# wen-yuan-zhang/Fast-Learning-NeRF

Hardware: AMD Instinct MI355X
Metric: training rays/sec (Lego-like 800x800, 64+128 samples) + PSNR@N-iters (higher is better)
Workload: dtype f32; 1 GPU; nerf-ours Lego full 800x800 (BASELINE configs[1]), SURVEY 8(d) throughput protocol: 4096 uniformly drawn rays per GPU per step, 64+128 samples, use_viewdirs, white_bkgd, perturb=1, U[0,1) targets, random-init nets, leaf-error table on, fp32-width bf16x6 kernels, plain backward (FASTNERF_COMPACT=0); parallelism=dp1, math_mode=bf16x6, backward=plain (every sample)

## Files before the change

fast-learning-nerf_amd/_lib.py:

```python
import ctypes as C
import os

import torch

HERE = os.path.dirname(os.path.abspath(__file__))
LIB_PATH = os.environ.get('FASTNERF_LIB') or os.path.join(HERE, 'libfastnerf.so')

P = C.c_void_p
I = C.c_int
L = C.c_int64
F = C.c_float
D = C.c_double
U64 = C.c_uint64



class StepArgs(C.Structure):
    _fields_ = (
        [('n', L)] + [(k, P) for k in ('rays_o', 'rays_d', 'target', 't_rand', 'u', 'noise0', 'noise1')]
        + [('seed0', U64), ('seed1', U64), ('leaf_tag', P), ('table', P), ('net_floats', L)]
        + [(k, P) for k in ('params', 'grads', 'adam_m', 'adam_v', 'packed_fwd_c', 'packed_bwd_c', 'packed_fwd_f', 'packed_bwd_f',
                            'rays11', 'z0', 'raw0', 'act0', 'rgb0', 'disp0', 'acc0', 'w0', 'depth0',
                            'z1', 'z_samples', 'z_std', 'raw1', 'act1', 'rgb1', 'disp1', 'acc1', 'w1', 'depth1',
                            'g_rgb', 'g_rgb0', 'loss2', 'draw_ws', 'act_ws', 'dact_ws', 'partial_ws', 'live_ws', 'counts')]
        + [(k, D) for k in ('focal', 'lr', 'beta1', 'beta2', 'eps')]
        + [(k, F) for k in ('near_plane', 'far_plane', 'grad_scale')]
        + [(k, I) for k in ('math_mode', 'N_samples', 'N_importance', 'lindisp', 'perturb', 'white_bkgd', 'ndc', 'H', 'W', 'live',
                            'fwd_flags', 'max_leaves', 'adam_t')]
        + [('occ', P), ('occ_counts', P)])


class OccGrid(C.Structure):
    _fields_ = [('words', P), ('lo', F * 3), ('inv', F * 3), ('n', C.c_int32 * 3), ('outside_occupied', C.c_int32)]


OCC_MAX_LEVELS = 8


class OccCascade(C.Structure):
    _fields_ = [('levels', C.c_int32), ('reserved', C.c_int32), ('level', OccGrid * OCC_MAX_LEVELS)]


STEP_FORWARD, STEP_BWD_FINE, STEP_BWD_COARSE, STEP_UPDATE = 1, 2, 4, 8

SIGNATURES = {
    'fastnerf_version': (I, []),
    'fastnerf_last_error': (C.c_char_p, []),
    'fastnerf_device_cus': (I, []),
    'fastnerf_gen_rays': (I, [I, I, F, F, F, F, P, P, P, P]),
    'fastnerf_gen_rays_pixels': (I, [L, P, P, F, F, F, F, P, P, P]),
    'fastnerf_ndc_rays': (I, [L, I, I, D, F, P, P, P, P, P]),
    'fastnerf_pack_rays': (I, [L, P, P, F, F, I, I, I, D, P, P]),
    'fastnerf_sample_coarse': (I, [L, I, P, I, I, P, U64, P, P]),
    'fastnerf_posenc': (I, [L, I, P, P, P]),
    'fastnerf_mlp_pack': (I, [P, P, P, P]),
    'fastnerf_mlp_fwd': (I, [L, I, P, P, P, P, P, P, P]),
    'fastnerf_mlp_bwd_partial_floats': (L, []),
    'fastnerf_mlp_bwd': (I, [L, I, P, P, P, P, P, P, P, P]),
    'fastnerf_raw2outputs_fwd': (I, [L, I, P, P, P, P, I, P, P, P, P, P, P]),
    'fastnerf_raw2outputs_bwd': (I, [L, I, P, P, P, P, I, P, P, P]),
    'fastnerf_raw2outputs_bwd_full': (I, [L, I, P, P, P, P, I, P, P, P, P, P, P, P, P, P]),
    'fastnerf_sample_pdf_merge': (I, [L, I, I, P, P, I, P, U64, P, P, P, P]),
    'fastnerf_sample_pdf': (I, [L, I, I, P, P, I, P, U64, P, P]),
    'fastnerf_mse_leafmax': (I, [L, P, P, P, F, P, P, P, P, I, P, P]),
    'fastnerf_adam_step': (I, [L, P, P, P, P, D, D, D, D, I, P]),
    'fastnerf_net_floats': (L, [I, I]),
    'fastnerf_mlp_act_floats': (L, [I, L]),
    'fastnerf_mlp_pack_ex': (I, [I, P, P, P, P]),
    'fastnerf_mlp_fwd_ex': (I, [I, L, I, P, P, P, P, P, P, P]),
    'fastnerf_mlp_bwd_ex': (I, [I, L, I, P, P, P, P, P, P, P, P]),
    'fastnerf_mlp_bf16_floats': (L, [I, I, L]),
    'fastnerf_mlp_bf16_partial_floats': (L, []),
    'fastnerf_mlp_bf16_pack': (I, [I, P, P, P, P]),
    'fastnerf_mlp_bf16_fwd': (I, [I, L, I, P, P, P, P, P, P, P]),
    'fastnerf_mlp_bf16_bwd': (I, [I, L, I, P, P, P, P, P, P, P, P]),
    'fastnerf_render_rays_fwd': (I, [I, L, I, I, P, I, I, I, I, P, P, P, P, U64, U64, P, P, P, P] + [P] * 18 + [P]),
    'fastnerf_render_rays_fwd_ex': (I, [I, L, I, I, P, I, I, I, I, P, P, P, P, U64, U64, P, P, P, P] + [P] * 18 + [I, P]),
    'fastnerf_mlp_bf16_fwd_flags': (I, [I, L, I, P, P, P, P, P, I, P]),
    'fastnerf_mlp_fwd_flags_ex': (I, [I, L, I, P, P, P, P, P, I, P]),
    'fastnerf_render_rays_bwd': (I, [I, L, I, I, P, I] + [P] * 20),
    'fastnerf_pp_intersect_sphere': (I, [L, P, P, P, P]),
    'fastnerf_pp_fg_depths': (I, [L, I, F, P, I, P, U64, P, P]),
    'fastnerf_pp_sample_pdf_merge': (I, [L, I, I, P, P, I, P, U64, P, P, P]),
    'fastnerf_pp_perturb_samples': (I, [L, I, P, P, U64, P, P]),
    'fastnerf_pp_sample_pdf': (I, [L, I, I, P, P, I, P, U64, P, P]),
    'fastnerf_pp_depth2pts_outside': (I, [L, I, P, P, P, P, P, P]),
    'fastnerf_pp_composite_fwd': (I, [L, I, I, P, P, P, P, P, P, P, P, P]),
    'fastnerf_pp_composite_bwd': (I, [L, I, I, P, P, P, P, P, P, P, P]),
    'fastnerf_pp_gen_rays': (I, [I, I, P, P, P, P, P]),
    'fastnerf_leaf_sumcount': (I, [L, P, P, P, I, P, P, P]),
    'fastnerf_tree_adjust_mean': (L, [P, P, P, I, D]),
    'fastnerf_tree_create': (P, [I, I, I, I]),
    'fastnerf_tree_destroy': (None, [P]),
    'fastnerf_tree_num_leaves': (I, [P, I]),
    'fastnerf_tree_max_leaves': (I, [P]),
    'fastnerf_tree_min_area': (D, [P, I]),
    'fastnerf_tree_get_leaves': (I, [P, I, P]),
    'fastnerf_tree_set_leaves': (I, [P, I, I, P, D]),
    'fastnerf_tree_leaf_plan': (I, [P, I, D, I, P]),
    'fastnerf_tree_adjust': (L, [P, P, I, D]),
    'fastnerf_tree_epoch_plan': (L, [P, D, I, P, P]),
    'fastnerf_epoch_rays': (I, [L, I, P, P, P, P, I, I, I, F, F, F, F, U64, I] + [P] * 10 + [P]),
    'fastnerf_epoch_rays_shard': (I, [L, I, P, P, P, P, I, I, I, F, F, F, F, U64, I] + [P] * 5 + [L, I, I] + [P] * 5 + [P]),
    'fastnerf_epoch_shard_rows': (L, [L, L, I, I]),
    'fastnerf_gauss_noise': (I, [L, F, U64, P, P]),
    'fastnerf_compact_ws_ints': (L, [L]),
    'fastnerf_compact_live': (I, [L, P, P, P, P, P]),
    'fastnerf_mlp_bf16_fwd_live': (I, [I, L, I, P, P, P, P, P, P, P, P]),
    'fastnerf_mlp_bf16_bwd_live': (I, [I, L, I, P, P, P, P, P, P, P, P, P, P]),
    'fastnerf_mlp_fwd_live_ex': (I, [I, L, I, P, P, P, P, P, P, P, P]),
    'fastnerf_mlp_bwd_live_ex': (I, [I, L, I, P, P, P, P, P, P, P, P, P, P]),
    'fastnerf_render_rays_bwd_live': (I, [I, L, I, I, P, I] + [P] * 22 + [P]),
    'fastnerf_mlp_x6_packed_floats': (L, [I, I]),
    'fastnerf_mlp_x6_pack': (I, [I, P, P, P, P]),
    'fastnerf_mlp_x6_fwd': (I, [I, L, I, P, P, P, P, P, P, I, P]),
    'fastnerf_mlp_x6_bwd': (I, [I, L, I, P, P, P, P, P, P, P, P]),
    'fastnerf_mlp_x6_fwd_live': (I, [I, L, I, P, P, P, P, P, P, P, P]),
    'fastnerf_mlp_x6_bwd_live': (I, [I, L, I, P, P, P, P, P, P, P, P, P, P]),
    'fastnerf_step_args_size': (L, []),
    'fastnerf_train_step': (I, [C.POINTER(StepArgs), I, P]),
    'fastnerf_comm_unique_id': (I, [C.c_char_p]),
    'fastnerf_comm_init': (I, [C.POINTER(P), C.c_char_p, I, I]),
    'fastnerf_comm_destroy': (I, [P]),
    'fastnerf_allreduce_grads': (I, [P, P, L, C.c_float, P]),
    'fastnerf_allreduce_leaf_table': (I, [P, P, L, P]),
    'fastnerf_allreduce_leaf_sumcount': (I, [P, P, P, L, P]),
    'fastnerf_leaf_table_reset': (I, [P, L, P]),
    'fastnerf_leaf_table_read': (I, [P, P, L, P]),
    'fastnerf_grid_points': (I, [L, L, P, L, P, L, P, L, P, P]),
    'fastnerf_grid_sigma': (I, [L, P, P, P]),
    'fastnerf_mc_ws_bytes': (L, [L, L, L]),
    'fastnerf_mc_count': (I, [P, L, L, L, F, P, P, P]),
    'fastnerf_mc_emit': (I, [P, L, L, L, F, P, P, P, P]),
    'fastnerf_mc_tables': (I, [P, P]),
    'fastnerf_occ_words': (L, [L, L, L]),
    'fastnerf_occ_build': (I, [P, L, L, L, F, I, P, P, P]),
    'fastnerf_occ_from_mask': (I, [P, L, L, L, P, P]),
    'fastnerf_occ_query': (I, [C.POINTER(OccGrid), L, P, P, P]),
    'fastnerf_occ_classify': (I, [C.POINTER(OccGrid), L, I, P, P, P, P, P, P, P]),
    'fastnerf_occ_query_cascade': (I, [C.POINTER(OccCascade), L, P, P, P]),
    'fastnerf_occ_classify_cascade': (I, [C.POINTER(OccCascade), L, I, P, P, P, P, P, P, P]),
    'fastnerf_occ_cell_points': (I, [C.POINTER(OccGrid), L, L, U64, P, P]),
    'fastnerf_occ_update': (I, [P, P, L, L, L, L, L, F, F, I, P, P, P, P]),
    'fastnerf_mlp_fwd_list_ex': (I, [I, L, I, P, P, P, P, P, P, P, I, P]),
    'fastnerf_mlp_bf16_fwd_list': (I, [I, L, I, P, P, P, P, P, P, P, I, P]),
    'fastnerf_mlp_x6_fwd_list': (I, [I, L, I, P, P, P, P, P, P, P, I, P]),
    'fastnerf_render_rays_fwd_occ': (I, [I, L, I, I, P, I, I, I, I, P, P, U64, U64, P, P, P, P, C.POINTER(OccGrid), P, P] + [P] * 16 + [I, P]),
    'fastnerf_render_rays_fwd_occ_cascade': (I, [I, L, I, I, P, I, I, I, I, P, P, U64, U64, P, P, P, P, C.POINTER(OccCascade), P, P] + [P] * 16 + [I, P]),
    'fastnerf_mlp_sigma_grad_ws_floats': (L, [I, L]),
    'fastnerf_mlp_sigma_grad': (I, [I, I, L, I, P, P, P, P, P, P, P, P, P]),
}

_lib = None


def lib():
    global _lib
    if _lib is None:
        if not os.path.exists(LIB_PATH):
            raise RuntimeError(
                f'{LIB_PATH} not found: build it with `python -c "import __graft_entry__ as g; g.build()"` '
                '(the HIP path has no CPU fallback)')
        l = C.CDLL(LIB_PATH)
        for name, (res, args) in SIGNATURES.items():
            fn = getattr(l, name)
            fn.restype = res
            fn.argtypes = args
        if l.fastnerf_step_args_size() != C.sizeof(StepArgs):
            raise RuntimeError('fn_step_args: the ctypes mirror does not match the library (stale libfastnerf.so?)')
        _lib = l
    return _lib


def check(rc, what):
    if rc is None or rc < 0:
        msg = lib().fastnerf_last_error()
        raise RuntimeError(f'{what} failed ({rc}): {msg.decode() if msg else "?"}')
    return rc


def ptr(t):
    if t is None:
        return None
    assert t.is_contiguous(), 'tensor must be contiguous'
    return t.data_ptr()


def stream():
    return torch.cuda.current_stream().cuda_stream


def require_gpu(*tensors):
    for t in tensors:
        if t is not None and not t.is_cuda:
            raise RuntimeError('fastnerf ops run on the GPU only (no CPU fallback): got a CPU tensor')
```

fast-learning-nerf_amd/csrc/mlp_bwd_dw.hip:

```cpp
#include "mlp_common.h"

int fn_launch_dx(int mm, int grid, hipStream_t st, int64_t P, const float* draw, const float* act, const float* params, const float* packed_bwd,
                 float* dact, const NetLayout& L, const int* live_idx, const int* live_cnt);

#define DW_MT 32

template <int WO, int WI, int TO, int TI, bool BIAS, bool RANK1>
__global__ void __launch_bounds__(WO * WI * 64, WO * WI / 4)
mlp_bwd_dw_kernel(int64_t P, const float* __restrict__ dY, int ldy, const float* __restrict__ X, int ldx,
                  const float* __restrict__ draw , float* __restrict__ partial_w,
                  float* __restrict__ partial_b, float* __restrict__ partial_r, const int* __restrict__ live_idx,
                  const int* __restrict__ live_cnt) {
  if (live_idx) P = (int64_t)__builtin_amdgcn_readfirstlane(*live_cnt);
  constexpr int NO = WO * TO * 32, KI = WI * TI * 32;
  constexpr int NTD = WO * WI * 64;
  constexpr int STAGE = DW_MT * (NO + KI) + DW_MT;
  extern __shared__ __attribute__((aligned(16))) float smem[];
  const int tid = threadIdx.x;
  const int lane = tid & 63;
  const int wave = __builtin_amdgcn_readfirstlane(tid >> 6);
  const int wo = wave / WI, wi = wave % WI;
  const int64_t ntile_all = (P + DW_MT - 1) / DW_MT;
  const int64_t per = (ntile_all + gridDim.x - 1) / gridDim.x;
  const int64_t t0 = blockIdx.x * per;
  int64_t t1 = t0 + per;
  if (t1 > ntile_all) t1 = ntile_all;

  f32x16 acc[TO][TI];
#pragma unroll
  for (int a = 0; a < TO; ++a)
#pragma unroll
    for (int b = 0; b < TI; ++b)
#pragma unroll
      for (int r = 0; r < 16; ++r) acc[a][b][r] = 0.f;
  float bsum = 0.f, rsum = 0.f;

  constexpr int YV = (DW_MT * NO / 4 + NTD - 1) / NTD;
  constexpr int XV = (DW_MT * KI / 4 + NTD - 1) / NTD;
  static_assert(DW_MT * NO % 4 == 0 && DW_MT * KI % 4 == 0 && NO <= NTD && KI <= NTD, "stage split");
  float4 ry[YV], rx[XV];
  float rda = 0.f;

  auto load_stage = [&](int64_t t) {
    const int64_t pbase = t * DW_MT;
#pragma unroll
    for (int i = 0; i < YV; ++i) {
      const int e = (i * NTD + tid) * 4;
      const int m = e / NO, c = e % NO;
      const int64_t p = pbase + m;
      ry[i] = (e < DW_MT * NO && p < P) ? *reinterpret_cast<const float4*>(dY + p * ldy + c)
                                        : make_float4(0.f, 0.f, 0.f, 0.f);
    }
#pragma unroll
    for (int i = 0; i < XV; ++i) {
      const int e = (i * NTD + tid) * 4;
      const int m = e / KI, c = e % KI;
      const int64_t p = pbase + m;
      rx[i] = (e < DW_MT * KI && p < P) ? *reinterpret_cast<const float4*>(X + p * ldx + c)
                                        : make_float4(0.f, 0.f, 0.f, 0.f);
    }
    if (RANK1 && tid < DW_MT) {
      const int64_t p = pbase + tid;
      rda = (p < P) ? draw[(live_idx ? (int64_t)live_idx[p] : p) * 4 + 3] : 0.f;
    }
  };
  auto store_stage = [&](float* st) {
#pragma unroll
    for (int i = 0; i < YV; ++i)
      if ((i * NTD + tid) * 4 < DW_MT * NO) *reinterpret_cast<float4*>(st + (i * NTD + tid) * 4) = ry[i];
#pragma unroll
    for (int i = 0; i < XV; ++i)
      if ((i * NTD + tid) * 4 < DW_MT * KI) *reinterpret_cast<float4*>(st + DW_MT * NO + (i * NTD + tid) * 4) = rx[i];
    if (RANK1 && tid < DW_MT) st[DW_MT * (NO + KI) + tid] = rda;
  };

  if (t0 < t1) {
    load_stage(t0);
    store_stage(smem);
  }
  __syncthreads();
  for (int64_t t = t0; t < t1; ++t) {
    float* cur = smem + ((t - t0) & 1) * STAGE;
    float* nxt = smem + (((t - t0) & 1) ^ 1) * STAGE;
    if (t + 1 < t1) load_stage(t + 1);
    const float* Ys = cur;
    const float* Xs = cur + DW_MT * NO;
    {
      float fa0[TO], fb0[TI], fa1[TO], fb1[TI];
      auto ldf = [&](float (&a)[TO], float (&b)[TI], int k2) {
        const int m = k2 * 2 + (lane >> 5);
#pragma unroll
        for (int i = 0; i < TO; ++i) a[i] = Ys[m * NO + (wo * TO + i) * 32 + (lane & 31)];
#pragma unroll
        for (int j = 0; j < TI; ++j) b[j] = Xs[m * KI + (wi * TI + j) * 32 + (lane & 31)];
      };
      auto mm = [&](const float (&a)[TO], const float (&b)[TI]) {
#pragma unroll
        for (int i = 0; i < TO; ++i)
#pragma unroll
          for (int j = 0; j < TI; ++j) acc[i][j] = mfma(a[i], b[j], acc[i][j]);
      };
      ldf(fa0, fb0, 0);
#pragma unroll
      for (int k2 = 0; k2 < DW_MT / 2; k2 += 2) {
        ldf(fa1, fb1, k2 + 1);
        __builtin_amdgcn_sched_barrier(0);
        mm(fa0, fb0);
        __builtin_amdgcn_sched_barrier(0);
        if (k2 + 2 < DW_MT / 2) ldf(fa0, fb0, k2 + 2);
        __builtin_amdgcn_sched_barrier(0);
        mm(fa1, fb1);
        __builtin_amdgcn_sched_barrier(0);
      }
    }
    if (BIAS) {
      if (tid < NO) {
#pragma unroll 8
        for (int m = 0; m < DW_MT; ++m) bsum += Ys[m * NO + tid];
      }
    }
    if (RANK1) {
      if (tid < KI) {
        const float* da = cur + DW_MT * (NO + KI);
#pragma unroll 8
        for (int m = 0; m < DW_MT; ++m) rsum = fmaf(da[m], Xs[m * KI + tid], rsum);
      }
    }
    if (t + 1 < t1) store_stage(nxt);
    __syncthreads();
  }
  float* pw = partial_w + (int64_t)blockIdx.x * NO * KI;
#pragma unroll
  for (int i = 0; i < TO; ++i)
#pragma unroll
    for (int j = 0; j < TI; ++j)
#pragma unroll
      for (int r = 0; r < 16; ++r) {
        const int o = (wo * TO + i) * 32 + crow(r, lane);
        const int c = (wi * TI + j) * 32 + (lane & 31);
        pw[(int64_t)o * KI + c] = acc[i][j][r];
      }
  if (BIAS && tid < NO) partial_b[(int64_t)blockIdx.x * NO + tid] = bsum;
  if (RANK1 && tid < KI) partial_r[(int64_t)blockIdx.x * KI + tid] = rsum;
}

template <int WO, int WI, int TO, int TI, bool BIAS, bool RANK1, int CTI2 = 0, int CTO2 = 0>
__device__ __forceinline__ void dw6_body(const int64_t P, const float* __restrict__ dY, const float* __restrict__ X,
                                         const float* __restrict__ draw, float* __restrict__ partial_w, float* __restrict__ partial_b,
                                         float* __restrict__ partial_r, const int* __restrict__ live_idx,
                                         const float* __restrict__ X2, const float* __restrict__ dY2, const int wg, const int nwg) {
  constexpr int NO = WO * TO * 32, KI = WI * TI * 32;
  constexpr int CTO = WO * TO, CTI = WI * TI, NTILE = CTO + CTI;
  constexpr int NW = WO * WI;
  constexpr int TPW = (NTILE + NW - 1) / NW;
  extern __shared__ __attribute__((aligned(16))) uint4 S6[];
  float* const DA = reinterpret_cast<float*>(S6 + 2 * NTILE * 192);
  const int tid = threadIdx.x;
  const int lane = tid & 63;
  const int wave = __builtin_amdgcn_readfirstlane(tid >> 6);
  const int wo = wave / WI, wi = wave % WI;
  const int64_t nq_all = (P + 15) / 16;
  const int64_t per = (nq_all + nwg - 1) / nwg;
  const int64_t q0 = wg * per;
  int64_t q1 = q0 + per;
  if (q1 > nq_all) q1 = nq_all;
  const int nq = (int)(q1 - q0);
  int64_t Pend = q1 * 16;
  if (Pend > P) Pend = P;

  f32x16 acc[TO][TI];
#pragma unroll
  for (int a = 0; a < TO; ++a)
#pragma unroll
    for (int b = 0; b < TI; ++b)
#pragma unroll
      for (int r = 0; r < 16; ++r) acc[a][b][r] = 0.f;
  float ssum[TPW];
#pragma unroll
  for (int k = 0; k < TPW; ++k) ssum[k] = 0.f;

  constexpr int CTI1 = CTI - CTI2, KI1 = CTI1 * 32, KI2 = CTI2 * 32;
  static_assert(!(RANK1 && CTI2), "the rank-1 row is taken over X only");
  constexpr int CTO1 = CTO - CTO2, NO1 = CTO1 * 32, NO2 = CTO2 * 32;
  static_assert(!(RANK1 && CTO2) && !(CTI2 && CTO2), "one second tensor per job");
  const float* tsrc[TPW];
  bool tisy[TPW], tis2[TPW];
  constexpr bool KNOWN = (CTO % NW == 0) && (NTILE % NW == 0) && CTO2 == 0 && CTI2 == 0;
#pragma unroll
  for (int k = 0; k < TPW; ++k) {
    const int t = k * NW + wave;
    tisy[k] = KNOWN ? (k * NW < CTO) : (t < CTO);
    tis2[k] = (CTI2 > 0 && t >= CTO + CTI1) || (CTO2 > 0 && t >= CTO1 && t < CTO);
    tsrc[k] = tisy[k] ? (tis2[k] ? dY2 + q0 * (16 * NO2) + (t - CTO1) * 32 : dY + q0 * (16 * NO1) + t * 32)
                      : (tis2[k] ? X2 + q0 * (16 * KI2) + (t - CTO - CTI1) * 32 : X + q0 * (16 * KI1) + (t - CTO) * 32);
  }
  const int relmax = (int)(Pend - q0 * 16) - 1;
  const int col = lane & 31, half8 = (lane >> 5) * 8;
  const unsigned boffy = (unsigned)(half8 * NO1 + col) * 4u, boffy2 = (unsigned)(half8 * NO2 + col) * 4u,
                 boffx = (unsigned)(half8 * KI1 + col) * 4u, boffx2 = (unsigned)(half8 * KI2 + col) * 4u;
  struct Raw { float v[TPW][8]; };
  auto ldb = [](const float* base, unsigned byte_off) __attribute__((always_inline)) -> float {
    return *reinterpret_cast<const float*>(reinterpret_cast<const char*>(base) + byte_off);
  };
  auto load_raw = [&](Raw& r, int st, auto whole) __attribute__((always_inline)) {
    if constexpr (decltype(whole)::value) {
#pragma unroll
      for (int k = 0; k < TPW; ++k) {
        const int t = k * NW + wave;
        if (NTILE % NW == 0 || t < NTILE) {
          if (tisy[k] && CTO2 > 0 && tis2[k]) {
            const float* b = tsrc[k] + (int64_t)st * (16 * NO2);
#pragma unroll
            for (int e = 0; e < 8; ++e) r.v[k][e] = ldb(b, boffy2 + (unsigned)(e * NO2 * 4));
          } else if (tisy[k]) {
            const float* b = tsrc[k] + (int64_t)st * (16 * NO1);
#pragma unroll
            for (int e = 0; e < 8; ++e) r.v[k][e] = ldb(b, boffy + (unsigned)(e * NO1 * 4));
          } else if (CTI2 > 0 && tis2[k]) {
            const float* b = tsrc[k] + (int64_t)st * (16 * KI2);
#pragma unroll
            for (int e = 0; e < 8; ++e) r.v[k][e] = ldb(b, boffx2 + (unsigned)(e * KI2 * 4));
          } else {
            const float* b = tsrc[k] + (int64_t)st * (16 * KI1);
#pragma unroll
            for (int e = 0; e < 8; ++e) r.v[k][e] = ldb(b, boffx + (unsigned)(e * KI1 * 4));
          }
        }
      }
    } else {
      unsigned row[8];
#pragma unroll
      for (int e = 0; e < 8; ++e) { const int rr = st * 16 + half8 + e; row[e] = (unsigned)(rr < relmax ? rr : relmax); }
#pragma unroll
      for (int k = 0; k < TPW; ++k) {
        const int t = k * NW + wave;
        if (NTILE % NW == 0 || t < NTILE) {
#pragma unroll
          for (int e = 0; e < 8; ++e)
            r.v[k][e] = ldb(tsrc[k], (row[e] * (unsigned)(tisy[k] ? (tis2[k] ? NO2 : NO1) : (tis2[k] ? KI2 : KI1)) + (unsigned)col) * 4u);
        }
      }
    }
  };
  const int* const li = live_idx ? live_idx : reinterpret_cast<const int*>(draw);
  auto load_ix = [&](int st) __attribute__((always_inline)) -> int64_t {
    const int rr = st * 16 + (lane & 15);
    const int64_t p = q0 * 16 + (rr < relmax ? rr : relmax);
    const int64_t lv = li[p];
    return live_idx ? lv : p;
  };
  auto split_store = [&](const Raw& r, int buf, int st, auto whole) __attribute__((always_inline)) {
    const int nv = relmax + 1 - (st * 16 + half8);
#pragma unroll
    for (int k = 0; k < TPW; ++k) {
      const int t = k * NW + wave;
      if (NTILE % NW == 0 || t < NTILE) {
        float v[8];
#pragma unroll
        for (int e = 0; e < 8; ++e) v[e] = r.v[k][e];
        if constexpr (!decltype(whole)::value) {
#pragma unroll
          for (int e = 0; e < 8; ++e) v[e] = e < nv ? v[e] : 0.f;
        }
        uint4 h, m, l;
        uint4* d = S6 + ((buf * NTILE + t) * 3) * 64 + lane;
        split3_frag(make_float4(v[0], v[1], v[2], v[3]), make_float4(v[4], v[5], v[6], v[7]), h, m, l);
        d[0] = h; d[64] = m; d[128] = l;
        if (BIAS && (KNOWN ? (k * NW < CTO) : (t < CTO1))) ssum[k] += ((v[0] + v[1]) + (v[2] + v[3])) + ((v[4] + v[5]) + (v[6] + v[7]));
        if (RANK1 && (KNOWN ? (k * NW >= CTO) : (t >= CTO))) {
          const float4 d0 = *reinterpret_cast<const float4*>(DA + (st & 1) * 16 + half8);
          const float4 d1 = *reinterpret_cast<const float4*>(DA + (st & 1) * 16 + half8 + 4);
          const float da[8] = {d0.x, d0.y, d0.z, d0.w, d1.x, d1.y, d1.z, d1.w};
#pragma unroll
          for (int e = 0; e < 8; ++e) ssum[k] = fmaf(da[e], v[e], ssum[k]);
        }
      }
    }
  };
  auto multiply = [&](int buf) __attribute__((always_inline)) {
    const uint4* Sb = S6 + buf * NTILE * 192 + lane;
    uint4 a[TO][3];
#pragma unroll
    for (int i = 0; i < TO; ++i)
#pragma unroll
      for (int pl = 0; pl < 3; ++pl) a[i][pl] = Sb[((wo * TO + i) * 3 + pl) * 64];
    constexpr int PA[6] = {2, 0, 1, 1, 0, 0}, PB[6] = {0, 2, 1, 0, 1, 0};
    constexpr int JP = TI >= 2 ? 2 : 1;
#pragma unroll
    for (int j0 = 0; j0 < TI; j0 += JP) {
      uint4 b[JP][3];
#pragma unroll
      for (int jj = 0; jj < JP; ++jj)
#pragma unroll
        for (int pl = 0; pl < 3; ++pl)
          if (j0 + jj < TI) b[jj][pl] = Sb[((CTO + wi * TI + j0 + jj) * 3 + pl) * 64];
#pragma unroll
      for (int t = 0; t < 6; ++t)
#pragma unroll
        for (int jj = 0; jj < JP; ++jj)
#pragma unroll
          for (int i = 0; i < TO; ++i)
            if (j0 + jj < TI) acc[i][j0 + jj] = mfma_bf16(a[i][PA[t]], b[jj][PB[t]], acc[i][j0 + jj]);
    }
  };
  auto publish = [&]() __attribute__((always_inline)) {
    asm volatile("s_waitcnt lgkmcnt(0)\n\ts_barrier" ::: "memory");
  };

  if (nq > 0) {
    constexpr std::true_type WHOLE{};
    constexpr std::false_type ANY{};
    Raw r0, r1;
    load_raw(r0, 0, ANY);
    load_raw(r1, 1, ANY);
    float dr0 = 0.f, dr1 = 0.f;
    int64_t ix0 = 0, ix1 = 0;
    const bool da_lane = RANK1 && wave == 0 && lane < 16;
    if (da_lane) {
      DA[lane] = draw[load_ix(0) * 4 + 3];
      DA[16 + lane] = draw[load_ix(1) * 4 + 3];
      dr0 = draw[load_ix(2) * 4 + 3];
      dr1 = draw[load_ix(3) * 4 + 3];
      ix0 = load_ix(4);
      ix1 = load_ix(5);
    }
    if (RANK1) publish();
    split_store(r0, 0, 0, ANY);
    load_raw(r0, 2, ANY);
    publish();
    auto mix = [&](auto sync) __attribute__((always_inline)) {
      if constexpr (KNOWN && !RANK1) interleave6<0, TO * TI * 6, TPW * 4 * 11 + (BIAS ? 8 : 0), decltype(sync)::value>();
    };
    auto pair = [&](int d, auto whole) __attribute__((always_inline)) {
      const int st = 2 * d;
      if (da_lane) { DA[lane] = dr0; dr0 = draw[ix0 * 4 + 3]; ix0 = load_ix(st + 6); }
      multiply(0);
      split_store(r1, 1, st + 1, whole);
      mix(std::integral_constant<int, 1>{});
      load_raw(r1, st + 3, whole);
      publish();
      if (da_lane) { DA[16 + lane] = dr1; dr1 = draw[ix1 * 4 + 3]; ix1 = load_ix(st + 7); }
      multiply(1);
      split_store(r0, 0, st + 2, whole);
      mix(std::integral_constant<int, 2>{});
      load_raw(r0, st + 4, whole);
      publish();
    };
    const int n2 = (nq + 1) / 2;
    const int nwhole = (relmax + 1) / 16;
    int dmain = nwhole >= 5 ? (nwhole - 3) / 2 : 0;
    if (dmain > n2) dmain = n2;
#pragma unroll 1
    for (int d = 0; d < dmain; ++d) pair(d, WHOLE);
#pragma unroll 1
    for (int d = dmain; d < n2; ++d) pair(d, ANY);
  }
  float* pw = partial_w + (int64_t)wg * NO * KI;
#pragma unroll
  for (int i = 0; i < TO; ++i)
#pragma unroll
    for (int j = 0; j < TI; ++j)
#pragma unroll
      for (int r = 0; r < 16; ++r) {
        const int o = (wo * TO + i) * 32 + crow(r, lane);
        const int c = (wi * TI + j) * 32 + (lane & 31);
        pw[(int64_t)o * KI + c] = acc[i][j][r];
      }
  if (BIAS || RANK1) {
#pragma unroll
    for (int k = 0; k < TPW; ++k) {
      const int t = k * NW + wave;
      if (NTILE % NW == 0 || t < NTILE) {
        const float sv = ssum[k] + __shfl_xor(ssum[k], 32, 64);
        if (lane < 32) {
          if (BIAS && t < CTO1) partial_b[(int64_t)wg * NO1 + t * 32 + lane] = sv;
          if (RANK1 && t >= CTO) partial_r[(int64_t)wg * KI + (t - CTO) * 32 + lane] = sv;
        }
      }
    }
  }
}

template <int WO, int WI, int TO, int TI, bool BIAS, bool RANK1, int CTI2 = 0, int CTO2 = 0>
__global__ void __launch_bounds__(WO * WI * 64, WO * WI / 4)
mlp_bwd_dw6_kernel(int64_t P, const float* __restrict__ dY, const float* __restrict__ X,
                   const float* __restrict__ draw, float* __restrict__ partial_w, float* __restrict__ partial_b,
                   float* __restrict__ partial_r, const int* __restrict__ live_idx, const int* __restrict__ live_cnt,
                   const float* __restrict__ X2 = nullptr, const float* __restrict__ dY2 = nullptr) {
  if (live_idx) P = (int64_t)__builtin_amdgcn_readfirstlane(*live_cnt);
  dw6_body<WO, WI, TO, TI, BIAS, RANK1, CTI2, CTO2>(P, dY, X, draw, partial_w, partial_b, partial_r, live_idx, X2, dY2, (int)blockIdx.x,
                                                    (int)gridDim.x);
}

#define DW_QMAX 256
__host__ __device__ static inline int dw_trunk_chunks(int64_t P, int ncu) {
  const int unit = ncu >= 8 ? ncu / 8 : 1;
  const int64_t nq = (P + 15) / 16;
  int64_t k = (nq + (int64_t)unit * DW_QMAX - 1) / ((int64_t)unit * DW_QMAX);
  k = k < 1 ? 1 : (k > 8 ? 8 : k);
  return unit * (int)k;
}
struct DwTrunk {
  const float* dY[8];
  const float* X[8];
  float* pw[8];
  float* pb[8];
};
__global__ void __launch_bounds__(512, 2)
mlp_bwd_dw6_trunk_kernel(int64_t P, DwTrunk J, const float* __restrict__ draw, float* __restrict__ partial_r,
                         const int* __restrict__ live_idx, const int* __restrict__ live_cnt, int ncu) {
  if (live_idx) P = (int64_t)__builtin_amdgcn_readfirstlane(*live_cnt);
  const int nact = dw_trunk_chunks(P, ncu);
  if ((int)blockIdx.x >= nact) return;
  const int job = (int)blockIdx.y;
  if (job == 7)
    dw6_body<4, 2, 2, 4, true, true>(P, J.dY[7], J.X[7], draw, J.pw[7], J.pb[7], partial_r, live_idx, nullptr, nullptr, (int)blockIdx.x, nact);
  else
    dw6_body<4, 2, 2, 4, true, false>(P, J.dY[job], J.X[job], nullptr, J.pw[job], J.pb[job], nullptr, live_idx, nullptr, nullptr,
                                      (int)blockIdx.x, nact);
}

__global__ void __launch_bounds__(128) head_grads_kernel(int64_t P, const float* __restrict__ draw,
                                                          const float* __restrict__ hv,
                                                          float* __restrict__ partial, const int* __restrict__ live_idx,
                                                          const int* __restrict__ live_cnt) {
  const int k = threadIdx.x;
  if (live_idx) P = *live_cnt;
  auto dptr = [&](int64_t q) { return draw + (live_idx ? (int64_t)live_idx[q] : q) * 4; };
  const int64_t per = (P + gridDim.x - 1) / gridDim.x;
  const int64_t pa = blockIdx.x * per;
  int64_t pb = pa + per;
  if (pb > P) pb = P;
  float s0 = 0.f, s1 = 0.f, s2 = 0.f, sb = 0.f;
  int64_t p = pa;
  constexpr int NF = 16;
  for (; p + NF <= pb; p += NF) {
    float4 d[NF];
    float h[NF];
#pragma unroll
    for (int i = 0; i < NF; ++i) {
      d[i] = *reinterpret_cast<const float4*>(dptr(p + i));
      h[i] = hv[(p + i) * 128 + k];
    }
#pragma unroll
    for (int i = 0; i < NF; ++i) {
      s0 = fmaf(d[i].x, h[i], s0); s1 = fmaf(d[i].y, h[i], s1); s2 = fmaf(d[i].z, h[i], s2);
      if (k < 4) sb += (k == 0) ? d[i].x : (k == 1) ? d[i].y : (k == 2) ? d[i].z : d[i].w;
    }
  }
  for (; p < pb; ++p) {
    const float4 d = *reinterpret_cast<const float4*>(dptr(p));
    const float h = hv[p * 128 + k];
    s0 = fmaf(d.x, h, s0); s1 = fmaf(d.y, h, s1); s2 = fmaf(d.z, h, s2);
    if (k < 4) sb += (k == 0) ? d.x : (k == 1) ? d.y : (k == 2) ? d.z : d.w;
  }
  float* o = partial + (int64_t)blockIdx.x * 388;
  o[k] = s0; o[128 + k] = s1; o[256 + k] = s2;
  if (k < 4) o[384 + k] = sb;
}

struct RedSeg {
  int64_t src;
  int64_t wg_stride;
  int64_t dst;
  int nwg, rows, cols, ld, valid_cols;
  int dyn;
};
#define MAX_SEGS 32
struct RedTable {
  RedSeg s[MAX_SEGS];
  int n;
};

__global__ void __launch_bounds__(256) reduce_all_kernel(RedTable tab, const float* __restrict__ partial,
                                                          float* __restrict__ grads, int64_t P, const int* __restrict__ live_cnt, int ncu) {
  RedSeg sg = tab.s[blockIdx.y];
  if (sg.dyn) {
    if (live_cnt) P = (int64_t)*live_cnt;
    const int n = dw_trunk_chunks(P, ncu);
    sg.nwg = n < sg.nwg ? n : sg.nwg;
  }
  const int64_t total = (int64_t)sg.rows * sg.cols;
  const float* src = partial + sg.src;
  for (int64_t e = blockIdx.x * (int64_t)blockDim.x + threadIdx.x; e < total; e += (int64_t)gridDim.x * blockDim.x) {
    const int r = (int)(e / sg.cols), c = (int)(e % sg.cols);
    if (c >= sg.valid_cols) continue;
    constexpr int RS = 16;
    float a[RS];
#pragma unroll
    for (int i = 0; i < RS; ++i) a[i] = 0.f;
    int w = 0;
    for (; w + RS <= sg.nwg; w += RS) {
#pragma unroll
      for (int i = 0; i < RS; ++i) a[i] += src[(int64_t)(w + i) * sg.wg_stride + e];
    }
#pragma unroll
    for (int i = 0; i < RS - 1; ++i)
      if (w + i < sg.nwg) a[i] += src[(int64_t)(w + i) * sg.wg_stride + e];
#pragma unroll
    for (int h = RS / 2; h >= 1; h >>= 1)
#pragma unroll
      for (int i = 0; i < h; ++i) a[i] += a[i + h];
    grads[sg.dst + (int64_t)r * sg.ld + c] = a[0];
  }
}

struct DwJobDesc { int NO, KI, bias, rank1; };
static DwJobDesc dw_job(int j, int pe_pad) {
  switch (j) {
    case 0: return {256, pe_pad, 1, 0};
    case 8: return {256, pe_pad, 0, 0};
    case 9: return {256, 256, 1, 1};
    case 10: return {128, 256, 1, 0};
    case 11: return {128, 32, 0, 0};
    default: return {256, 256, 1, 0};
  }
}
#define HEAD_MAX_WG 1024
static int64_t dw_job_floats(int j, int pe_pad) {
  const DwJobDesc d = dw_job(j, pe_pad);
  return (int64_t)d.NO * d.KI + (d.bias ? d.NO : 0) + (d.rank1 ? d.KI : 0);
}
static int64_t dw_job_base(int j, int ncu, int pe_pad) {
  static const int order[12] = {0, 8, 1, 2, 3, 4, 5, 6, 7, 9, 10, 11};
  int64_t o = 0;
  for (int i = 0; i < 12; ++i) {
    if (order[i] == j) return o;
    o += dw_job_floats(order[i], pe_pad) * ncu;
  }
  return o;
}
extern "C" int64_t fastnerf_mlp_bwd_partial_floats(void) {
  return dw_job_base(12, num_cus(), 96) + (int64_t)HEAD_MAX_WG * 388;
}

template <int WO, int WI, int TO, int TI, bool BIAS, bool RANK1, int MM = MM_F32, int CTI2 = 0, int CTO2 = 0>
static int launch_dw(int64_t P, const float* dY, int ldy, const float* X, int ldx, const float* draw, float* base,
                     int nwg, hipStream_t st, const int* live_idx = nullptr, const int* live_cnt = nullptr,
                     const float* X2 = nullptr, const float* dY2 = nullptr) {
  constexpr int NO = WO * TO * 32, KI = WI * TI * 32;
  float* pw = base;
  float* pb = base + (int64_t)nwg * NO * KI;
  float* pr = pb + (BIAS ? (int64_t)nwg * (NO - CTO2 * 32) : 0);
  if constexpr (MM == MM_X6) {
    if (ldy != NO - CTO2 * 32 || ldx != KI - CTI2 * 32 || (CTI2 > 0) != (X2 != nullptr) || (CTO2 > 0) != (dY2 != nullptr)) {
      fn::set_error("launch_dw: the bf16x6 dW kernel needs ld == width (and X2 / dY2 exactly when CTI2 / CTO2 > 0)");
      return -1;
    }
    constexpr int lds6 = 2 * (WO * TO + WI * TI) * 3 * 1024 + 128;
    auto kern6 = mlp_bwd_dw6_kernel<WO, WI, TO, TI, BIAS, RANK1, CTI2, CTO2>;
    static bool attr6 = false;
    if (!attr6) {
      FN_HIP(hipFuncSetAttribute(reinterpret_cast<const void*>(kern6), hipFuncAttributeMaxDynamicSharedMemorySize, lds6));
      attr6 = true;
    }
    hipLaunchKernelGGL(kern6, dim3(nwg), dim3(WO * WI * 64), lds6, st, P, dY, X, draw, pw, pb, pr, live_idx, live_cnt, X2, dY2);
    FN_LAUNCH_CHECK();
    return 0;
  } else {
    static_assert(MM == MM_F32 && CTI2 == 0 && CTO2 == 0, "two-tensor jobs exist for the bf16x6 dW kernel only");
    constexpr int STAGE = DW_MT * (NO + KI) + DW_MT;
    const size_t lds = 2 * STAGE * sizeof(float);
    auto kern = mlp_bwd_dw_kernel<WO, WI, TO, TI, BIAS, RANK1>;
    static bool attr = false;
    if (!attr) {
      FN_HIP(hipFuncSetAttribute(reinterpret_cast<const void*>(kern), hipFuncAttributeMaxDynamicSharedMemorySize, (int)lds));
      attr = true;
    }
    hipLaunchKernelGGL(kern, dim3(nwg), dim3(WO * WI * 64), lds, st, P, dY, ldy, X, ldx, draw, pw, pb, pr, live_idx, live_cnt);
    FN_LAUNCH_CHECK();
    return 0;
  }
}

static void add_seg(RedTable& T, int64_t src, int64_t wg_stride, int nwg, int rows, int cols, int64_t dst, int ld,
                    int valid_cols, int dyn = 0) {
  RedSeg& s = T.s[T.n++];
  s.src = src; s.wg_stride = wg_stride; s.nwg = nwg; s.rows = rows; s.cols = cols; s.dst = dst; s.ld = ld;
  s.valid_cols = valid_cols; s.dyn = dyn;
}

template <int MM>
static int bwd_launch_t(int kind, int64_t n, int S, const float* draw, const float* act, const float* params,
                      const float* packed_bwd, float* dact, float* partial, float* grads, const int* live_idx,
                      const int* live_cnt, fn_stream_t stream) {
  constexpr int MW = MM;
  const NetLayout& L = layout_of(kind);
  const int PEP = L.pe_pad;
  hipStream_t st = fn::S(stream);
  const int64_t P = n * S;
  const int64_t ntiles = (P + TM - 1) / TM;
  const int ncu = num_cus();
  int grid = ncu * WG_PER_CU;
  if (ntiles < grid) grid = (int)ntiles;
  if (int rc_dx = fn_launch_dx(MM, grid, st, P, draw, act, params, packed_bwd, dact, L, live_idx, live_cnt)) return rc_dx;

  const int nwg = ncu;
  RedTable T;
  T.n = 0;
  int rc;
  const float* a_pe = act + act_pe(P, PEP);
  auto region = [&](int j) { return partial + dw_job_base(j, ncu, PEP); };
  auto segs = [&](int j, int64_t dstW, int ld, int validc, int64_t dstB, int64_t dstR, int dyn = 0) {
    const DwJobDesc d = dw_job(j, PEP);
    const int64_t b = dw_job_base(j, ncu, PEP);
    add_seg(T, b, (int64_t)d.NO * d.KI, nwg, d.NO, d.KI, dstW, ld, validc, dyn);
    int64_t o = b + (int64_t)nwg * d.NO * d.KI;
    if (d.bias) { add_seg(T, o, d.NO, nwg, 1, d.NO, dstB, d.NO, d.NO, dyn); o += (int64_t)nwg * d.NO; }
    if (d.rank1) add_seg(T, o, d.KI, nwg, 1, d.KI, dstR, d.KI, d.KI, dyn);
  };
  if constexpr (MW == MM_X6) {
    if (PEP == 64) rc = launch_dw<8, 2, 2, 1, true, false, MW, 0, 8>(P, dact + dact_y(P, 0), 256, a_pe, 64, nullptr, region(0), nwg, st, live_idx, live_cnt, nullptr, dact + dact_y(P, 5));
    else rc = launch_dw<8, 1, 2, 3, true, false, MW, 0, 8>(P, dact + dact_y(P, 0), 256, a_pe, 96, nullptr, region(0), nwg, st, live_idx, live_cnt, nullptr, dact + dact_y(P, 5));
    if (rc) return rc;
    const int64_t b0 = dw_job_base(0, ncu, PEP);
    add_seg(T, b0, (int64_t)512 * PEP, nwg, 256, PEP, L.LW[0], L.in_pe, L.in_pe);
    add_seg(T, b0 + (int64_t)256 * PEP, (int64_t)512 * PEP, nwg, 256, PEP, L.LW[5], 256 + L.in_pe, L.in_pe);
    add_seg(T, b0 + (int64_t)nwg * 512 * PEP, 256, nwg, 1, 256, L.LB[0], 256, 256);
  } else {
    if (PEP == 64) rc = launch_dw<4, 1, 2, 2, true, false, MW>(P, dact + dact_y(P, 0), 256, a_pe, 64, nullptr, region(0), nwg, st, live_idx, live_cnt);
    else rc = launch_dw<4, 1, 2, 3, true, false, MW>(P, dact + dact_y(P, 0), 256, a_pe, 96, nullptr, region(0), nwg, st, live_idx, live_cnt);
    if (rc) return rc;
    segs(0, L.LW[0], L.in_pe, L.in_pe, L.LB[0], 0);
  }
  if constexpr (MW != MM_X6) {
    for (int l = 1; l < 8; ++l) {
      if ((rc = launch_dw<4, 2, 2, 4, true, false, MW>(P, dact + dact_y(P, l), 256, act + act_h(P, PEP, l - 1), 256, nullptr, region(l), nwg, st, live_idx, live_cnt))) return rc;
      segs(l, L.LW[l] + (l == 5 ? L.in_pe : 0), l == 5 ? 256 + L.in_pe : 256, 256, L.LB[l], 0);
    }
  }
  if constexpr (MW != MM_X6) {
    if (PEP == 64) rc = launch_dw<4, 1, 2, 2, false, false, MW>(P, dact + dact_y(P, 5), 256, a_pe, 64, nullptr, region(8), nwg, st, live_idx, live_cnt);
    else rc = launch_dw<4, 1, 2, 3, false, false, MW>(P, dact + dact_y(P, 5), 256, a_pe, 96, nullptr, region(8), nwg, st, live_idx, live_cnt);
    if (rc) return rc;
    segs(8, L.LW[5], 256 + L.in_pe, L.in_pe, 0, 0);
  }
  if constexpr (MW == MM_X6) {
    DwTrunk J;
    for (int l = 1; l <= 8; ++l) {
      const int j = l < 8 ? l : 9;
      J.dY[l - 1] = l < 8 ? dact + dact_y(P, l) : dact + dact_feat(P);
      J.X[l - 1] = act + act_h(P, PEP, l - 1);
      J.pw[l - 1] = region(j);
      J.pb[l - 1] = region(j) + (int64_t)nwg * 256 * 256;
    }
    float* pr = J.pb[7] + (int64_t)nwg * 256;
    constexpr int lds6 = 2 * 16 * 3 * 1024 + 128;
    static bool attr_t = false;
    if (!attr_t) {
      FN_HIP(hipFuncSetAttribute(reinterpret_cast<const void*>(mlp_bwd_dw6_trunk_kernel), hipFuncAttributeMaxDynamicSharedMemorySize, lds6));
      attr_t = true;
    }
    hipLaunchKernelGGL(mlp_bwd_dw6_trunk_kernel, dim3(dw_trunk_chunks(P, ncu), 8), dim3(512), lds6, st, P, J, draw, pr, live_idx, live_cnt, ncu);
    FN_LAUNCH_CHECK();
    for (int l = 1; l < 8; ++l) segs(l, L.LW[l] + (l == 5 ? L.in_pe : 0), l == 5 ? 256 + L.in_pe : 256, 256, L.LB[l], 0, 1);
    segs(9, L.FW, 256, 256, L.FB, L.AW, 1);
  } else {
    if ((rc = launch_dw<4, 2, 2, 4, true, true, MW>(P, dact + dact_feat(P), 256, act + act_h(P, PEP, 7), 256, draw, region(9), nwg, st, live_idx, live_cnt))) return rc;
    segs(9, L.FW, 256, 256, L.FB, L.AW);
  }
  if constexpr (MW == MM_X6) {
    if ((rc = launch_dw<4, 3, 1, 3, true, false, MW, 1, 0>(P, dact + dact_yv(P), 128, act + act_feat(P, PEP), 256, nullptr, region(10), nwg, st,
                                                     live_idx, live_cnt, act + act_vpe(P, PEP), nullptr))) return rc;
    const int64_t b10 = dw_job_base(10, ncu, PEP);
    add_seg(T, b10, 128 * 288, nwg, 128, 288, L.VW, 283, 283);
    add_seg(T, b10 + (int64_t)nwg * 128 * 288, 128, nwg, 1, 128, L.VB, 128, 128);
  } else {
    if ((rc = launch_dw<2, 4, 2, 2, true, false, MW>(P, dact + dact_yv(P), 128, act + act_feat(P, PEP), 256, nullptr, region(10), nwg, st, live_idx, live_cnt))) return rc;
    segs(10, L.VW, 283, 256, L.VB, 0);
    if ((rc = launch_dw<4, 1, 1, 1, false, false, MW>(P, dact + dact_yv(P), 128, act + act_vpe(P, PEP), 32, nullptr, region(11), nwg, st, live_idx, live_cnt))) return rc;
    segs(11, L.VW + 256, 283, 27, 0, 0);
  }
  {
    const int hg = HEAD_MAX_WG;
    const int64_t hb = dw_job_base(12, ncu, PEP);
    hipLaunchKernelGGL(head_grads_kernel, dim3(hg), dim3(128), 0, st, P, draw, act + act_hv(P, PEP), partial + hb, live_idx, live_cnt);
    FN_LAUNCH_CHECK();
    add_seg(T, hb, 388, hg, 1, 388, L.RW, 388, 387);
    add_seg(T, hb + 387, 388, hg, 1, 1, L.AB, 1, 1);
  }
  hipLaunchKernelGGL(reduce_all_kernel, dim3(256, T.n), dim3(256), 0, st, T, partial, grads, P, live_cnt, ncu);
  FN_LAUNCH_CHECK();
  return 0;
}
static int bwd_launch(int kind, int64_t n, int S, const float* draw, const float* act, const float* params,
                      const float* packed_bwd, float* dact, float* partial, float* grads, const int* live_idx,
                      const int* live_cnt, fn_stream_t stream, int mm = MM_F32) {
  return mm == MM_X6 ? bwd_launch_t<MM_X6>(kind, n, S, draw, act, params, packed_bwd, dact, partial, grads, live_idx, live_cnt, stream)
                     : bwd_launch_t<MM_F32>(kind, n, S, draw, act, params, packed_bwd, dact, partial, grads, live_idx, live_cnt, stream);
}
extern "C" int fastnerf_mlp_bwd_ex(int kind, int64_t n, int S, const float* draw, const float* act,
                                   const float* params, const float* packed_bwd, float* dact, float* partial,
                                   float* grads, fn_stream_t stream) {
  FN_CHECK_ARG(kind >= 0 && kind <= 2 && n > 0 && S >= 1, "kind in 0..2, n>0, S>=1");
  FN_CHECK_ARG(draw && act && params && packed_bwd && dact && partial && grads, "null pointer");
  return bwd_launch(kind, n, S, draw, act, params, packed_bwd, dact, partial, grads, nullptr, nullptr, stream);
}
extern "C" int fastnerf_mlp_bwd_live_ex(int kind, int64_t n, int S, const float* draw, const float* act,
                                        const float* params, const float* packed_bwd, float* dact, float* partial,
                                        float* grads, const int32_t* live_idx, const int32_t* live_cnt,
                                        fn_stream_t stream) {
  FN_CHECK_ARG(kind >= 0 && kind <= 2 && n > 0 && S >= 1, "kind in 0..2, n>0, S>=1");
  FN_CHECK_ARG(draw && act && params && packed_bwd && dact && partial && grads && live_idx && live_cnt, "null pointer");
  return bwd_launch(kind, n, S, draw, act, params, packed_bwd, dact, partial, grads, live_idx, live_cnt, stream);
}
extern "C" int fastnerf_mlp_bwd(int64_t n, int S, const float* draw, const float* act, const float* params,
                                const float* packed_bwd, float* dact, float* partial, float* grads,
                                fn_stream_t stream) {
  return fastnerf_mlp_bwd_ex(0, n, S, draw, act, params, packed_bwd, dact, partial, grads, stream);
}

extern "C" int fastnerf_mlp_x6_bwd(int kind, int64_t n, int S, const float* draw, const float* act, const float* params,
                                   const float* packed_bwd, float* dact, float* partial, float* grads, fn_stream_t stream) {
  FN_CHECK_ARG(kind >= 0 && kind <= 2 && n > 0 && S >= 1, "kind in 0..2, n>0, S>=1");
  FN_CHECK_ARG(draw && act && params && packed_bwd && dact && partial && grads, "null pointer");
  return bwd_launch(kind, n, S, draw, act, params, packed_bwd, dact, partial, grads, nullptr, nullptr, stream, MM_X6);
}
extern "C" int fastnerf_mlp_x6_bwd_live(int kind, int64_t n, int S, const float* draw, const float* act, const float* params,
                                        const float* packed_bwd, float* dact, float* partial, float* grads,
                                        const int32_t* live_idx, const int32_t* live_cnt, fn_stream_t stream) {
  FN_CHECK_ARG(kind >= 0 && kind <= 2 && n > 0 && S >= 1, "kind in 0..2, n>0, S>=1");
  FN_CHECK_ARG(draw && act && params && packed_bwd && dact && partial && grads && live_idx && live_cnt, "null pointer");
  return bwd_launch(kind, n, S, draw, act, params, packed_bwd, dact, partial, grads, live_idx, live_cnt, stream, MM_X6);
}
```

fast-learning-nerf_amd/csrc/mlp_bwd_dx.hip:

```cpp
#include "mlp_common.h"

struct DxPre {
  unsigned mlo, mhi;
  float wan[4];
};
template <bool MASK, bool RANK1, bool L16 = false>
__device__ __forceinline__ DxPre dx_preload(const unsigned long long* __restrict__ maskw, const float* __restrict__ wa,
                                            int wn, int lane) {
  DxPre p;
  p.mlo = p.mhi = 0u;
  p.wan[0] = p.wan[1] = p.wan[2] = p.wan[3] = 0.f;
  if (MASK) {
    const unsigned long long w = maskw[lane];
    p.mlo = (unsigned)w;
    p.mhi = (unsigned)(w >> 32);
  }
  if (RANK1) {
    if constexpr (L16) {
#pragma unroll
      for (int ct = 0; ct < 4; ++ct) p.wan[ct] = wa[(wn * 4 + ct) * 16 + (lane & 15)];
    } else {
      p.wan[0] = wa[(wn * 2 + 0) * 32 + (lane & 31)];
      p.wan[1] = wa[(wn * 2 + 1) * 32 + (lane & 31)];
    }
  }
  return p;
}
template <bool MASK, bool RANK1>
__device__ __forceinline__ void epilogue_dx(const f32x4m (&acc)[4][4], float* Hs, const float* Es_dalpha, const DxPre& pre,
                                            float* __restrict__ dsave, int wm, int wn, int lane, int valid) {
  asm volatile("" : "+v"(lane));
  const unsigned mlo = pre.mlo, mhi = pre.mhi;
  float* colp[4][4];
  h_cols16<4>(Hs, wm, wn, lane, colp);
  const int hq = lane >> 4;
#pragma unroll
  for (int mt = 0; mt < 4; ++mt) {
#pragma unroll
    for (int ct = 0; ct < 4; ++ct) {
      const float wan = pre.wan[ct];
#pragma unroll
      for (int r = 0; r < 4; ++r) {
        float v = acc[mt][ct][r];
        if (RANK1) v = fmaf(Es_dalpha[wm * 64 + mt * 16 + 4 * hq + r], wan, v);
        if (MASK) {
          const int idx = (mt * 4 + ct) * 4 + r;
          const int keep = __builtin_amdgcn_sbfe(idx < 32 ? (int)mlo : (int)mhi, 31 - (idx & 31), 1);
          v = __int_as_float(__float_as_int(v) & keep);
        }
        H16_AT(colp, ct, mt, r) = v;
      }
    }
    __builtin_amdgcn_sched_barrier(0);
  }
}

template <bool MASK, bool RANK1>
__device__ __forceinline__ void epilogue_dx(const f32x16 (&acc)[2][2], float* Hs, const float* Es_dalpha,
                                            const DxPre& pre, float* __restrict__ dsave, int wm, int wn, int lane,
                                            int valid) {
  asm volatile("" : "+v"(lane));
  const unsigned mlo = pre.mlo, mhi = pre.mhi;
  float* colp[2][8];
  h_cols<2>(Hs, wm, wn, lane, colp);
#pragma unroll
  for (int nt = 0; nt < 2; ++nt) {
    const int n = (wn * 2 + nt) * 32 + (lane & 31);
    const float wan = pre.wan[nt];
#pragma unroll
    for (int mt = 0; mt < 2; ++mt) {
#pragma unroll
      for (int r = 0; r < 16; ++r) {
        const int m = wm * 64 + mt * 32 + crow(r, lane);
        float v = acc[mt][nt][r];
        if (RANK1) v = fmaf(Es_dalpha[m], wan, v);
        if (MASK) {
          const int idx = (nt * 2 + mt) * 16 + r;
          const int keep = __builtin_amdgcn_sbfe(idx < 32 ? (int)mlo : (int)mhi, 31 - (idx & 31), 1);
          v = __int_as_float(__float_as_int(v) & keep);
        }
        H_AT(colp, nt, mt, r) = v;
        if (dsave != nullptr && m < valid) dsave[(unsigned)(m * 256 + n)] = v;
      }
      __builtin_amdgcn_sched_barrier(0);
    }
  }
}

template <int MM = MM_F32>
__global__ void __launch_bounds__(NTHR, 2 * NTHR / 512 * WG_PER_CU)
mlp_bwd_dx_kernel(int64_t P, const float* __restrict__ draw, const float* __restrict__ act,
                  const float* __restrict__ params, const float* __restrict__ packed_t, float* __restrict__ dact,
                  NetLayout lay, unsigned* __restrict__ sched, const int* __restrict__ live_idx,
                  const int* __restrict__ live_cnt) {
  const int64_t PL = P;
  if (live_idx) P = (int64_t)__builtin_amdgcn_readfirstlane(*live_cnt);
  extern __shared__ __attribute__((aligned(16))) float smem[];
  float* Hs = smem;
  float* Es = smem + LDS_H;
  volatile int* sched_word = reinterpret_cast<volatile int*>(Es + 1024);
  const int tid = threadIdx.x;
  const int lane = tid & 63;
  const int wave = __builtin_amdgcn_readfirstlane(tid >> 6);
  const int wm = wave >> 2, wn = wave & 3;
  const int64_t ntiles = (P + TM - 1) / TM;
  stagger_start();

  for (int64_t tile = blockIdx.x; tile < ntiles;) {
    const int64_t p0 = tile * TM;
    const int valid = (int)((P - p0) < TM ? (P - p0) : TM);
    const unsigned long long* maskw =
        reinterpret_cast<const unsigned long long*>(act + act_mask(PL, lay.pe_pad)) + tile * (8 * NWAVES * 64);
    {
      const int pm = tid >> 2, pq = tid & 3;
      const bool ok = pm < valid;
      const int64_t pp = ok ? p0 + pm : P - 1;
      const float4 dr = *reinterpret_cast<const float4*>(draw + (live_idx ? (int64_t)live_idx[pp] : pp) * 4);
      if (pq == 0) Es[pm] = ok ? dr.w : 0.f;
      const float* wr = params + lay.RW;
      const float* hv = act + act_hv(PL, lay.pe_pad) + pp * 128;
      float* dyv = dact + dact_yv(PL) + pp * 128;
#pragma unroll
      for (int i = 0; i < 8; ++i) {
        const int k = pq * 32 + i * 4;
        const float4 h = *reinterpret_cast<const float4*>(hv + k);
        const float4 w0 = *reinterpret_cast<const float4*>(wr + k);
        const float4 w1 = *reinterpret_cast<const float4*>(wr + 128 + k);
        const float4 w2 = *reinterpret_cast<const float4*>(wr + 256 + k);
        float4 o;
        o.x = (h.x > 0.f) ? fmaf(dr.z, w2.x, fmaf(dr.y, w1.x, dr.x * w0.x)) : 0.f;
        o.y = (h.y > 0.f) ? fmaf(dr.z, w2.y, fmaf(dr.y, w1.y, dr.x * w0.y)) : 0.f;
        o.z = (h.z > 0.f) ? fmaf(dr.z, w2.z, fmaf(dr.y, w1.z, dr.x * w0.z)) : 0.f;
        o.w = (h.w > 0.f) ? fmaf(dr.z, w2.w, fmaf(dr.y, w1.w, dr.x * w0.w)) : 0.f;
        if (!ok) o = make_float4(0.f, 0.f, 0.f, 0.f);
        *reinterpret_cast<float4*>(Hs + pm * 256 + ((((k >> 2) ^ (pm & 15))) << 2)) = o;
        if (ok) store_nt(dyv + k, o);
      }
    }
    __syncthreads();
    constexpr bool L16 = MM != MM_F32;
    constexpr bool CHAIN = L16;
    AccT<L16, 2> acc;
    WRegsT<L16, 2> wch;
    zero_acc<2>(acc);
    gemm<MM, 2, 0>(acc, Hs, 0, 16, wblock<MM>(packed_t, lay.PB[0]), 16, 0, wn * 2, wm, lane);
    __syncthreads();
    wprefetch(wch, wblock<MM>(packed_t, lay.PB[1]), 32, 0, 32, wn * 2, lane);
    epilogue_dx<false, false>(acc, Hs, Es, dx_preload<false, false, L16>(nullptr, nullptr, wn, lane), nullptr, wm, wn, lane,
                              valid);
    __syncthreads();
    zero_acc<2>(acc);
    {
      const DxPre pre = dx_preload<true, true, L16>(maskw + (7 * NWAVES + wave) * 64, params + lay.AW, wn, lane);
      gemm<MM, 2, 0, CHAIN>(acc, Hs, 0, 32, wblock<MM>(packed_t, lay.PB[1]), 32, 0, wn * 2, wm, lane, 0,
                            dact + dact_feat(PL) + p0 * 256, valid, wave, wch);
      __syncthreads();
      wprefetch(wch, wblock<MM>(packed_t, lay.PB[2]), 32, 0, 32, wn * 2, lane);
      epilogue_dx<true, true>(acc, Hs, Es, pre, nullptr, wm, wn, lane, valid);
    }
    __syncthreads();
#pragma unroll 1
    for (int l = 7; l >= 1; --l) {
      const int64_t off = lay.PB[9 - l];
      zero_acc<2>(acc);
      const DxPre pre = dx_preload<true, false, L16>(maskw + ((l - 1) * NWAVES + wave) * 64, nullptr, wn, lane);
      gemm<MM, 2, 0, CHAIN>(acc, Hs, 0, 32, wblock<MM>(packed_t, off), 32, 0, wn * 2, wm, lane, 0,
                            dact + dact_y(PL, l) + p0 * 256, valid, wave, wch);
      __syncthreads();
      wprefetch(wch, wblock<MM>(packed_t, lay.PB[l > 1 ? 10 - l : 8]), 32, 0, 32, wn * 2, lane);
      epilogue_dx<true, false>(acc, Hs, Es, pre, nullptr, wm, wn, lane, valid);
      __syncthreads();
    }
    {
      float* d0 = dact + dact_y(PL, 0) + p0 * 256;
      for (int i = tid; i < TM * 64; i += NTHR) {
        const int m = i >> 6, sl = i & 63;
        if (m < valid)
          store_nt(d0 + m * 256 + ((sl ^ (m & 15)) << 2), *reinterpret_cast<const float4*>(Hs + m * 256 + sl * 4));
      }
    }
    tile = b_next_tile(sched, sched_word, tid);
  }
  b_sched_exit(sched, tid);
}

template <int MM>
static int launch_dx_t(int grid, hipStream_t st, int64_t P, const float* draw, const float* act, const float* params, const float* packed_bwd,
                       float* dact, const NetLayout& L, const int* live_idx, const int* live_cnt) {
  static bool attr_done = false;
  if (!attr_done) {
    FN_HIP(hipFuncSetAttribute(reinterpret_cast<const void*>(&mlp_bwd_dx_kernel<MM>),
                               hipFuncAttributeMaxDynamicSharedMemorySize, LDS_BYTES));
    attr_done = true;
  }
  unsigned* sched = b_sched_pair();
  FN_CHECK_ARG(sched != nullptr, "scheduler counters (hipMalloc failed?)");
  hipLaunchKernelGGL(mlp_bwd_dx_kernel<MM>, dim3(grid), dim3(NTHR), LDS_BYTES, st, P, draw, act, params, packed_bwd, dact, L, sched, live_idx, live_cnt);
  FN_LAUNCH_CHECK();
  return 0;
}
int fn_launch_dx(int mm, int grid, hipStream_t st, int64_t P, const float* draw, const float* act, const float* params, const float* packed_bwd,
                 float* dact, const NetLayout& L, const int* live_idx, const int* live_cnt) {
  return mm == MM_X6 ? launch_dx_t<MM_X6>(grid, st, P, draw, act, params, packed_bwd, dact, L, live_idx, live_cnt)
                     : launch_dx_t<MM_F32>(grid, st, P, draw, act, params, packed_bwd, dact, L, live_idx, live_cnt);
}
int fn_launch_dx_alone(int mm, int kind, int64_t P, const float* draw, const float* act, const float* params, const float* packed_bwd,
                       float* dact, hipStream_t st) {
  const int64_t ntiles = (P + TM - 1) / TM;
  int grid = num_cus() * WG_PER_CU;
  if (ntiles < grid) grid = (int)ntiles;
  return fn_launch_dx(mm, grid, st, P, draw, act, params, packed_bwd, dact, layout_of(kind), nullptr, nullptr);
}
```

fast-learning-nerf_amd/csrc/mlp_fwd.hip:

```cpp
#include "mlp_common.h"

__device__ __forceinline__ void bg_point(const float* __restrict__ o, const float* __restrict__ d, float depth,
                                         float x[4]) {
  const float dd = fadd(fadd(fmul(d[0], d[0]), fmul(d[1], d[1])), fmul(d[2], d[2]));
  const float od = fadd(fadd(fmul(d[0], o[0]), fmul(d[1], o[1])), fmul(d[2], o[2]));
  const float d1 = -od / dd;
  float pm_[3], ps[3];
#pragma unroll
  for (int c = 0; c < 3; ++c) pm_[c] = fadd(o[c], fmul(d1, d[c]));
  const float pmn = sqrtf(fadd(fadd(fmul(pm_[0], pm_[0]), fmul(pm_[1], pm_[1])), fmul(pm_[2], pm_[2])));
  const float dcos = 1.0f / sqrtf(dd);
  const float d2 = fmul(sqrtf(fsub(1.0f, fmul(pmn, pmn))), dcos);
  const float d12 = fadd(d1, d2);
#pragma unroll
  for (int c = 0; c < 3; ++c) ps[c] = fadd(o[c], fmul(d12, d[c]));
  float ax[3] = {fsub(fmul(o[1], ps[2]), fmul(o[2], ps[1])), fsub(fmul(o[2], ps[0]), fmul(o[0], ps[2])),
                 fsub(fmul(o[0], ps[1]), fmul(o[1], ps[0]))};
  const float an = sqrtf(fadd(fadd(fmul(ax[0], ax[0]), fmul(ax[1], ax[1])), fmul(ax[2], ax[2])));
#pragma unroll
  for (int c = 0; c < 3; ++c) ax[c] = ax[c] / an;
  const float ang = fsub(asinf(pmn), asinf(fmul(pmn, depth)));
  const float ca = cosf(ang), sa = sinf(ang);
  const float cr[3] = {fsub(fmul(ax[1], ps[2]), fmul(ax[2], ps[1])), fsub(fmul(ax[2], ps[0]), fmul(ax[0], ps[2])),
                       fsub(fmul(ax[0], ps[1]), fmul(ax[1], ps[0]))};
  const float dot = fadd(fadd(fmul(ax[0], ps[0]), fmul(ax[1], ps[1])), fmul(ax[2], ps[2]));
  const float omc = fsub(1.0f, ca);
  float pn[3];
#pragma unroll
  for (int c = 0; c < 3; ++c) pn[c] = fadd(fadd(fmul(ps[c], ca), fmul(cr[c], sa)), fmul(fmul(ax[c], dot), omc));
  const float nn = sqrtf(fadd(fadd(fmul(pn[0], pn[0]), fmul(pn[1], pn[1])), fmul(pn[2], pn[2])));
  x[0] = pn[0] / nn; x[1] = pn[1] / nn; x[2] = pn[2] / nn; x[3] = depth;
}

__device__ __forceinline__ int x2idx(int m, int k) { return m * 32 + ((((k >> 2) ^ ((m >> 1) & 7)) << 2) | (k & 3)); }

#define FN_SIN(a) (ABL_NOPE ? (a) : sinf(a))
#define FN_COS(a) (ABL_NOPE ? (a) : cosf(a))
template <bool SAVE, bool BG, int MM = MM_F32, bool LIST = false>
__global__ void __launch_bounds__(NTHR, 2 * NTHR / 512 * WG_PER_CU)
mlp_fwd_kernel(int64_t P, int S, const float* __restrict__ rays, const float* __restrict__ zv,
               const float* __restrict__ params, const float* __restrict__ packed, float* __restrict__ raw,
               float* __restrict__ act, NetLayout lay, unsigned* __restrict__ sched, const int* __restrict__ live_idx,
               const int* __restrict__ live_cnt, int flags) {
  const int64_t PL = P;
  if (live_idx) P = (int64_t)__builtin_amdgcn_readfirstlane(*live_cnt);
  extern __shared__ __attribute__((aligned(16))) float smem[];
  float* Hs = smem;
  float* Es = smem + LDS_H;
  float* X2 = smem;
  volatile int* sched_word = reinterpret_cast<volatile int*>(smem + LDS_H - 2);
  const int tid = threadIdx.x;
  const int lane = tid & 63;
  const int wave = __builtin_amdgcn_readfirstlane(tid >> 6);
  const int wm = wave >> 2, wn = wave & 3;
  const int64_t ntiles = (P + TM - 1) / TM;
  const int PEP = BG ? 96 : 64;
  const int dbg = 0;
  stagger_start();

  for (int64_t tile = blockIdx.x; tile < ntiles;) {
    const int64_t p0 = tile * TM;
    const int valid = (int)((P - p0) < TM ? (P - p0) : TM);
    unsigned long long* maskw =
        SAVE ? reinterpret_cast<unsigned long long*>(act + act_mask(PL, PEP)) + tile * (8 * NWAVES * 64) : nullptr;
    const int pm = tid >> 2, pq = tid & 3;
    int64_t pp = p0 + pm;
    if (pp >= P) pp = P - 1;
    if (live_idx) pp = live_idx[pp];
    const int64_t ray = pp / S;
    const float* rr = rays + ray * 11;
    float x4[4] = {0.f, 0.f, 0.f, 0.f};
    auto write_x2 = [&]() {
      const float xv = x4[pq];
      X2[x2idx(pm, 0 + pq)] = FN_COS(fmul(xv, 128.0f));
      X2[x2idx(pm, 4 + pq)] = FN_SIN(fmul(xv, 256.0f));
      X2[x2idx(pm, 8 + pq)] = FN_COS(fmul(xv, 256.0f));
      X2[x2idx(pm, 12 + pq)] = FN_SIN(fmul(xv, 512.0f));
      X2[x2idx(pm, 16 + pq)] = FN_COS(fmul(xv, 512.0f));
      X2[x2idx(pm, 20 + pq)] = 0.f; X2[x2idx(pm, 24 + pq)] = 0.f; X2[x2idx(pm, 28 + pq)] = 0.f;
    };
    if (!BG) {
      const float zz = zv[pp];
      float x[3];
#pragma unroll
      for (int c = 0; c < 3; ++c) x[c] = fadd(rr[c], fmul(rr[3 + c], zz));
      if (pq == 0) {
        Es[eidx(pm, 0)] = x[0]; Es[eidx(pm, 1)] = x[1]; Es[eidx(pm, 2)] = x[2];
        Es[eidx(pm, 63)] = 0.f;
      }
      for (int j = pq; j < 30; j += 4) {
        const int k = j / 3, dim = j - 3 * k;
        const float a = fmul(x[dim], (float)(1 << k));
        Es[eidx(pm, 3 + 6 * k + dim)] = FN_SIN(a);
        Es[eidx(pm, 6 + 6 * k + dim)] = FN_COS(a);
      }
    } else {
      const int sidx = (int)(pp - ray * S);
      const float zz = zv[ray * S + (S - 1 - sidx)];
      bg_point(rr, rr + 3, zz, x4);
      const float xv = x4[pq];
      Es[eidx(pm, pq)] = xv;
#pragma unroll
      for (int k = 0; k < 7; ++k) {
        const float a = fmul(xv, (float)(1 << k));
        Es[eidx(pm, 4 + 8 * k + pq)] = FN_SIN(a);
        Es[eidx(pm, 8 + 8 * k + pq)] = FN_COS(a);
      }
      Es[eidx(pm, 60 + pq)] = FN_SIN(fmul(xv, 128.0f));
      write_x2();
    }
    __syncthreads();
    if (SAVE) {
      float* ape = act + act_pe(PL, PEP) + p0 * PEP;
      for (int i = tid; i < TM * 16; i += NTHR) {
        const int m = i >> 4, sl = i & 15;
        if (m < valid)
          store_nt(ape + m * PEP + sl * 4, *reinterpret_cast<const float4*>(Es + m * 64 + ((sl ^ (m & 15)) << 2)));
      }
      if (BG) {
        for (int i = tid; i < TM * 8; i += NTHR) {
          const int m = i >> 3, sl = i & 7;
          if (m < valid)
            store_nt(ape + m * PEP + 64 + sl * 4,
                     *reinterpret_cast<const float4*>(X2 + m * 32 + ((sl ^ ((m >> 1) & 7)) << 2)));
        }
      }
    }
    constexpr bool L16 = MM != MM_F32;
    constexpr bool FOLD = L16;
    AccT<L16, 2> acc;
    constexpr int KS5 = (BG ? 96 + 256 : 64 + 256) / 8;
    float bv2[L16 ? 4 : 2];
    load_bias<2>(bv2, params + lay.LB[0], wn, lane);
    init_acc<2, FOLD>(acc, bv2);
    gemm<MM, 2, 1>(acc, Es, 0, 8, wblock<MM>(packed, lay.PF[0]), PEP / 8, 0, wn * 2, wm, lane, dbg);
    if (BG) {
      gemm<MM, 2, 2>(acc, X2, 0, 4, wblock<MM>(packed, lay.PF[0]), PEP / 8, 8, wn * 2, wm, lane, dbg);
      __syncthreads();
    }
    epilogue_fwd<2, true, SAVE, FOLD>(acc, bv2, Hs, wm, wn, lane, nullptr, 256, valid,
                                      SAVE ? maskw + (0 * NWAVES + wave) * 64 : nullptr);
    __syncthreads();
#pragma unroll 1
    for (int l = 1; l < 8; ++l) {
      const void* B = wblock<MM>(packed, lay.PF[l]);
      load_bias<2>(bv2, params + lay.LB[l], wn, lane);
      init_acc<2, FOLD>(acc, bv2);
      float* sv = SAVE ? act + act_h(PL, PEP, l - 1) + p0 * 256 : nullptr;
      if (l == 5) {
        if (!BG) {
          gemm<MM, 2, 1>(acc, Es, 0, 8, B, KS5, 0, wn * 2, wm, lane, dbg);
          gemm<MM, 2, 0>(acc, Hs, 0, 32, B, KS5, 8, wn * 2, wm, lane, dbg, sv, valid, wave);
        } else {
          gemm<MM, 2, 0>(acc, Hs, 0, 32, B, KS5, 12, wn * 2, wm, lane, dbg, sv, valid, wave);
          __syncthreads();
          write_x2();
          __syncthreads();
          gemm<MM, 2, 1>(acc, Es, 0, 8, B, KS5, 0, wn * 2, wm, lane, dbg);
          gemm<MM, 2, 2>(acc, X2, 0, 4, B, KS5, 8, wn * 2, wm, lane, dbg);
        }
      } else {
        gemm<MM, 2, 0>(acc, Hs, 0, 32, B, 32, 0, wn * 2, wm, lane, dbg, sv, valid, wave);
      }
      __syncthreads();
      epilogue_fwd<2, true, SAVE, FOLD>(acc, bv2, Hs, wm, wn, lane, nullptr, 256, valid,
                                        SAVE ? maskw + (l * NWAVES + wave) * 64 : nullptr);
      __syncthreads();
    }
    float alpha_val = 0.f;
    {
      const float* wa = params + lay.AW;
      float s = 0.f;
#pragma unroll
      for (int i = 0; i < 16; ++i) {
        const int k = pq * 64 + i * 4;
        const float4 h = *reinterpret_cast<const float4*>(Hs + pm * 256 + ((((k >> 2) ^ (pm & 15))) << 2));
        const float4 w = *reinterpret_cast<const float4*>(wa + k);
        s = fmaf(h.x, w.x, s); s = fmaf(h.y, w.y, s); s = fmaf(h.z, w.z, s); s = fmaf(h.w, w.w, s);
      }
      s += __shfl_xor(s, 1, 64);
      s += __shfl_xor(s, 2, 64);
      alpha_val = s + params[lay.AB];
      float v[3] = {rr[8], rr[9], rr[10]};
      if (pq == 0) {
        Es[eidx(pm, 0)] = v[0]; Es[eidx(pm, 1)] = v[1]; Es[eidx(pm, 2)] = v[2];
#pragma unroll
        for (int c = 27; c < 32; ++c) Es[eidx(pm, c)] = 0.f;
      }
      for (int j = pq; j < 12; j += 4) {
        const int k = j / 3, dim = j - 3 * k;
        const float a = fmul(v[dim], (float)(1 << k));
        Es[eidx(pm, 3 + 6 * k + dim)] = FN_SIN(a);
        Es[eidx(pm, 6 + 6 * k + dim)] = FN_COS(a);
      }
    }
    bool skip_tail = false;
    if (!SAVE && !BG && (flags & 1)) {
      const unsigned long long any_live = __ballot((pm < valid) && (alpha_val > 0.f));
      volatile int* slot = reinterpret_cast<volatile int*>(Es + 56);
      if (lane == 0) slot[wave] = any_live != 0ull;
      __syncthreads();
      int any = 0;
#pragma unroll
      for (int w = 0; w < NWAVES; ++w) any |= slot[w];
      skip_tail = any == 0;
    }
    if (skip_tail) {
      if (pq == 0 && pm < valid && raw) *reinterpret_cast<float4*>(raw + (LIST ? pp : p0 + pm) * 4) = make_float4(0.f, 0.f, 0.f, alpha_val);
    } else {
    load_bias<2>(bv2, params + lay.FB, wn, lane);
    init_acc<2, FOLD>(acc, bv2);
    gemm<MM, 2, 0>(acc, Hs, 0, 32, wblock<MM>(packed, lay.PF[8]), 32, 0, wn * 2, wm, lane, dbg,
                   SAVE ? act + act_h(PL, PEP, 7) + p0 * 256 : nullptr, valid, wave);
    __syncthreads();
    epilogue_fwd<2, false, false, FOLD>(acc, bv2, Hs, wm, wn, lane, nullptr, 256, valid);
    __syncthreads();
    if (SAVE) {
      float* avp = act + act_vpe(PL, PEP) + p0 * 32;
      for (int i = tid; i < TM * 8; i += NTHR) {
        const int m = i >> 3, sl = i & 7;
        if (m < valid)
          store_nt(avp + m * 32 + sl * 4, *reinterpret_cast<const float4*>(Es + m * 64 + ((sl ^ (m & 15)) << 2)));
      }
    }
    {
      AccT<L16, 1> av;
      float bv1[L16 ? 2 : 1];
      load_bias<1>(bv1, params + lay.VB, wn, lane);
      init_acc<1, FOLD>(av, bv1);
      gemm<MM, 1, 0>(av, Hs, 0, 32, wblock<MM>(packed, lay.PF[9]), 36, 0, wn, wm, lane, dbg,
                     SAVE ? act + act_feat(PL, PEP) + p0 * 256 : nullptr, valid, wave);
      gemm<MM, 1, 1>(av, Es, 0, 4, wblock<MM>(packed, lay.PF[9]), 36, 32, wn, wm, lane, dbg);
      __syncthreads();
      epilogue_fwd<1, true, false, FOLD>(av, bv1, Hs, wm, wn, lane, nullptr, 128, valid);
      __syncthreads();
      if (SAVE) {
        float* ahv = act + act_hv(PL, PEP) + p0 * 128;
        for (int i = tid; i < TM * 32; i += NTHR) {
          const int m = i >> 5, sl = i & 31;
          if (m < valid)
            store_nt(ahv + m * 128 + ((sl ^ (m & 15)) << 2), *reinterpret_cast<const float4*>(Hs + m * 256 + sl * 4));
        }
      }
    }
    {
      const float* wr = params + lay.RW;
      float s0 = 0.f, s1 = 0.f, s2 = 0.f;
#pragma unroll
      for (int i = 0; i < 8; ++i) {
        const int k = pq * 32 + i * 4;
        const float4 h = *reinterpret_cast<const float4*>(Hs + pm * 256 + ((((k >> 2) ^ (pm & 15))) << 2));
        const float4 w0 = *reinterpret_cast<const float4*>(wr + k);
        const float4 w1 = *reinterpret_cast<const float4*>(wr + 128 + k);
        const float4 w2 = *reinterpret_cast<const float4*>(wr + 256 + k);
        s0 = fmaf(h.x, w0.x, s0); s0 = fmaf(h.y, w0.y, s0); s0 = fmaf(h.z, w0.z, s0); s0 = fmaf(h.w, w0.w, s0);
        s1 = fmaf(h.x, w1.x, s1); s1 = fmaf(h.y, w1.y, s1); s1 = fmaf(h.z, w1.z, s1); s1 = fmaf(h.w, w1.w, s1);
        s2 = fmaf(h.x, w2.x, s2); s2 = fmaf(h.y, w2.y, s2); s2 = fmaf(h.z, w2.z, s2); s2 = fmaf(h.w, w2.w, s2);
      }
      s0 += __shfl_xor(s0, 1, 64); s0 += __shfl_xor(s0, 2, 64);
      s1 += __shfl_xor(s1, 1, 64); s1 += __shfl_xor(s1, 2, 64);
      s2 += __shfl_xor(s2, 1, 64); s2 += __shfl_xor(s2, 2, 64);
      if (pq == 0 && pm < valid && raw) {
        float4 o;
        o.x = s0 + params[lay.RB]; o.y = s1 + params[lay.RB + 1]; o.z = s2 + params[lay.RB + 2]; o.w = alpha_val;
        *reinterpret_cast<float4*>(raw + (LIST ? pp : p0 + pm) * 4) = o;
      }
    }
    }
    tile = b_next_tile(sched, sched_word, tid);
  }
  b_sched_exit(sched, tid);
}

template <bool SAVE, bool BG, int MM, bool LIST = false>
static int fwd_launch_t(int grid, hipStream_t st, int64_t P, int S, const float* rays11, const float* z, const float* params,
                        const float* packed_fwd, float* raw, float* act, const NetLayout& lay, unsigned* sched, const int* live_idx,
                        const int* live_cnt, int flags) {
  auto kern = mlp_fwd_kernel<SAVE, BG, MM, LIST>;
  static bool attr = false;
  if (!attr) {
    FN_HIP(hipFuncSetAttribute(reinterpret_cast<const void*>(kern), hipFuncAttributeMaxDynamicSharedMemorySize, LDS_BYTES));
    attr = true;
  }
  hipLaunchKernelGGL(kern, dim3(grid), dim3(NTHR), LDS_BYTES, st, P, S, rays11, z, params, packed_fwd, raw, act, lay, sched, live_idx,
                     live_cnt, flags);
  FN_LAUNCH_CHECK();
  return 0;
}

static int fwd_launch(int kind, int64_t n, int S, const float* rays11, const float* z, const float* params,
                      const float* packed_fwd, float* raw, float* act, const int* live_idx, const int* live_cnt,
                      fn_stream_t stream, int flags = 0, int mm = MM_F32) {
  const NetLayout& lay = layout_of(kind);
  const int64_t P = n * S;
  const int64_t ntiles = (P + TM - 1) / TM;
  int grid = num_cus() * WG_PER_CU;
  if (ntiles < grid) grid = (int)ntiles;
  hipStream_t st = fn::S(stream);
  unsigned* sched = b_sched_pair();
  FN_CHECK_ARG(sched != nullptr, "scheduler counters (hipMalloc failed?)");
  const int fl = (kind == 0 && !act && (!live_idx || raw)) ? flags : 0;
  if (live_idx && !act)
    return mm == MM_X6 ? fwd_launch_t<false, false, MM_X6, true>(grid, st, P, S, rays11, z, params, packed_fwd, raw, nullptr, lay, sched, live_idx, live_cnt, fl)
                       : fwd_launch_t<false, false, MM_F32, true>(grid, st, P, S, rays11, z, params, packed_fwd, raw, nullptr, lay, sched, live_idx, live_cnt, fl);
#define FN_FWD(SAVE_, BG_, MM_) \
  fwd_launch_t<SAVE_, BG_, MM_>(grid, st, P, S, rays11, z, params, packed_fwd, raw, act, lay, sched, live_idx, live_cnt, fl)
  if (mm == MM_X6) {
    if (kind == 2) return act ? FN_FWD(true, true, MM_X6) : FN_FWD(false, true, MM_X6);
    return act ? FN_FWD(true, false, MM_X6) : FN_FWD(false, false, MM_X6);
  }
  if (kind == 2) return act ? FN_FWD(true, true, MM_F32) : FN_FWD(false, true, MM_F32);
  return act ? FN_FWD(true, false, MM_F32) : FN_FWD(false, false, MM_F32);
#undef FN_FWD
}
extern "C" int fastnerf_mlp_fwd_ex(int kind, int64_t n, int S, const float* rays11, const float* z,
                                   const float* params, const float* packed_fwd, float* raw, float* act,
                                   fn_stream_t stream) {
  FN_CHECK_ARG(kind >= 0 && kind <= 2 && n >= 0 && S >= 1, "kind in 0..2, n>=0, S>=1");
  FN_CHECK_ARG(n == 0 || (rays11 && z && params && packed_fwd && raw), "null pointer");
  if (n == 0) return 0;
  return fwd_launch(kind, n, S, rays11, z, params, packed_fwd, raw, act, nullptr, nullptr, stream);
}
extern "C" int fastnerf_mlp_fwd_flags_ex(int kind, int64_t n, int S, const float* rays11, const float* z, const float* params,
                                         const float* packed_fwd, float* raw, int flags, fn_stream_t stream) {
  FN_CHECK_ARG(kind >= 0 && kind <= 2 && n >= 0 && S >= 1, "kind in 0..2, n>=0, S>=1");
  FN_CHECK_ARG(n == 0 || (rays11 && z && params && packed_fwd && raw), "null pointer");
  if (n == 0) return 0;
  return fwd_launch(kind, n, S, rays11, z, params, packed_fwd, raw, nullptr, nullptr, nullptr, stream, flags);
}

extern "C" int fastnerf_mlp_fwd_live_ex(int kind, int64_t n, int S, const float* rays11, const float* z,
                                        const float* params, const float* packed_fwd, float* act,
                                        const int32_t* live_idx, const int32_t* live_cnt, fn_stream_t stream) {
  FN_CHECK_ARG(kind >= 0 && kind <= 2 && n > 0 && S >= 1, "kind in 0..2, n>0, S>=1");
  FN_CHECK_ARG(rays11 && z && params && packed_fwd && act && live_idx && live_cnt, "null pointer");
  FN_CHECK_ARG(n * (int64_t)S < ((int64_t)1 << 31), "live lists index points with int32");
  return fwd_launch(kind, n, S, rays11, z, params, packed_fwd, nullptr, act, live_idx, live_cnt, stream);
}
extern "C" int fastnerf_mlp_fwd(int64_t n, int S, const float* rays11, const float* z, const float* params,
                                const float* packed_fwd, float* raw, float* act, fn_stream_t stream) {
  return fastnerf_mlp_fwd_ex(0, n, S, rays11, z, params, packed_fwd, raw, act, stream);
}

extern "C" int fastnerf_mlp_x6_fwd(int kind, int64_t n, int S, const float* rays11, const float* z, const float* params,
                                   const float* packed_fwd, float* raw, float* act, int flags, fn_stream_t stream) {
  FN_CHECK_ARG(kind >= 0 && kind <= 2 && n >= 0 && S >= 1, "kind in 0..2, n>=0, S>=1");
  FN_CHECK_ARG(n == 0 || (rays11 && z && params && packed_fwd && raw), "null pointer");
  if (n == 0) return 0;
  return fwd_launch(kind, n, S, rays11, z, params, packed_fwd, raw, act, nullptr, nullptr, stream, flags, MM_X6);
}
extern "C" int fastnerf_mlp_x6_fwd_live(int kind, int64_t n, int S, const float* rays11, const float* z, const float* params,
                                        const float* packed_fwd, float* act, const int32_t* live_idx, const int32_t* live_cnt,
                                        fn_stream_t stream) {
  FN_CHECK_ARG(kind >= 0 && kind <= 2 && n > 0 && S >= 1, "kind in 0..2, n>0, S>=1");
  FN_CHECK_ARG(rays11 && z && params && packed_fwd && act && live_idx && live_cnt, "null pointer");
  FN_CHECK_ARG(n * (int64_t)S < ((int64_t)1 << 31), "live lists index points with int32");
  return fwd_launch(kind, n, S, rays11, z, params, packed_fwd, nullptr, act, live_idx, live_cnt, stream, 0, MM_X6);
}

extern "C" int fastnerf_mlp_fwd_list_ex(int kind, int64_t n, int S, const float* rays11, const float* z, const float* params,
                                        const float* packed_fwd, float* raw, const int32_t* live_idx, const int32_t* live_cnt,
                                        int flags, fn_stream_t stream) {
  FN_CHECK_ARG(kind == 0 && n > 0 && S >= 1, "kind == 0, n>0, S>=1");
  FN_CHECK_ARG(rays11 && z && params && packed_fwd && raw && live_idx && live_cnt, "null pointer");
  FN_CHECK_ARG(n * (int64_t)S < ((int64_t)1 << 31), "lists index points with int32");
  return fwd_launch(kind, n, S, rays11, z, params, packed_fwd, raw, nullptr, live_idx, live_cnt, stream, flags);
}
extern "C" int fastnerf_mlp_x6_fwd_list(int kind, int64_t n, int S, const float* rays11, const float* z, const float* params,
                                        const float* packed_fwd, float* raw, const int32_t* live_idx, const int32_t* live_cnt,
                                        int flags, fn_stream_t stream) {
  FN_CHECK_ARG(kind == 0 && n > 0 && S >= 1, "kind == 0, n>0, S>=1");
  FN_CHECK_ARG(rays11 && z && params && packed_fwd && raw && live_idx && live_cnt, "null pointer");
  FN_CHECK_ARG(n * (int64_t)S < ((int64_t)1 << 31), "lists index points with int32");
  return fwd_launch(kind, n, S, rays11, z, params, packed_fwd, raw, nullptr, live_idx, live_cnt, stream, flags, MM_X6);
}
```

fast-learning-nerf_amd/csrc/mlp_layout.h:

```cpp
#pragma once
#include <stdint.h>

namespace fnl {
struct NetLayout {
  int64_t LW[8], LB[8];
  int64_t VW, VB, FW, FB, AW, AB, RW, RB;
  int64_t PF[10], PB[9];
  int64_t n_params, pf_total, pb_total;
  int in_pe, pe_pad;
  int kind;
};

inline NetLayout make_layout(int kind) {
  NetLayout L{};
  L.kind = kind;
  L.in_pe = (kind == 2) ? 84 : 63;
  L.pe_pad = (kind == 2) ? 96 : 64;
  int64_t o = 0;
  for (int i = 0; i < 8; ++i) {
    const int fan = (i == 0) ? L.in_pe : (i == 5 ? 256 + L.in_pe : 256);
    L.LW[i] = o; o += (int64_t)256 * fan;
    L.LB[i] = o; o += 256;
  }
  auto V = [&]() { L.VW = o; o += 128 * 283; L.VB = o; o += 128; };
  auto F = [&]() { L.FW = o; o += 256 * 256; L.FB = o; o += 256; };
  auto A = [&]() { L.AW = o; o += 256; L.AB = o; o += 1; };
  auto R = [&]() { L.RW = o; o += 3 * 128; L.RB = o; o += 3; };
  if (kind == 0) { V(); F(); A(); R(); } else { A(); F(); V(); R(); }
  L.n_params = o;
  int64_t p = 0;
  for (int l = 0; l < 10; ++l) {
    L.PF[l] = p;
    const int kp = (l == 0) ? L.pe_pad : (l == 5 ? L.pe_pad + 256 : (l == 9 ? 288 : 256));
    p += (int64_t)kp * (l == 9 ? 128 : 256);
  }
  L.pf_total = p;
  p = 0;
  for (int j = 0; j < 9; ++j) { L.PB[j] = p; p += (int64_t)(j == 0 ? 128 : 256) * 256; }
  L.pb_total = p;
  return L;
}

constexpr int ACT_REST = 8 * 256 + 256 + 32 + 128;
constexpr int ACT_MASK = 64;
inline __host__ __device__ int64_t act_pe(int64_t P, int pe_pad) { return 0; }
inline __host__ __device__ int64_t act_h(int64_t P, int pe_pad, int l) { return P * pe_pad + (int64_t)l * P * 256; }
inline __host__ __device__ int64_t act_feat(int64_t P, int pe_pad) { return P * (pe_pad + 2048); }
inline __host__ __device__ int64_t act_vpe(int64_t P, int pe_pad) { return P * (pe_pad + 2048 + 256); }
inline __host__ __device__ int64_t act_hv(int64_t P, int pe_pad) { return P * (pe_pad + 2048 + 256 + 32); }
inline __host__ __device__ int64_t act_mask(int64_t P, int pe_pad) { return P * (pe_pad + ACT_REST); }
inline int64_t act_floats(int64_t P, int pe_pad) { return P * (pe_pad + ACT_REST + ACT_MASK) + 8192; }
constexpr int DACT_FLOATS = 8 * 256 + 256 + 128;
inline __host__ __device__ int64_t dact_y(int64_t P, int l) { return (int64_t)l * P * 256; }
inline __host__ __device__ int64_t dact_feat(int64_t P) { return 8 * P * 256; }
inline __host__ __device__ int64_t dact_yv(int64_t P) { return 9 * P * 256; }
}
```

fast-learning-nerf_amd/csrc/mlp_pack.hip:

```cpp
#include "mlp_common.h"

struct PackDesc {
  int64_t src_off;
  int64_t dst_off;
  int ld;
  int n_rows;
  int n_cols;
  int segA_pad, segA_valid, segB_valid;
  int col0;
  int transposed;
};
struct PackTable {
  PackDesc d[19];
};

__global__ void __launch_bounds__(256) pack_kernel(PackTable tab, const float* __restrict__ params,
                                                    float* __restrict__ pf, float* __restrict__ pb) {
  const PackDesc d = tab.d[blockIdx.y];
  const int64_t total = (int64_t)d.n_rows * d.n_cols;
  float* dst = (d.transposed ? pb : pf) + d.dst_off;
  const float* src = params + d.src_off;
  for (int64_t e = blockIdx.x * (int64_t)blockDim.x + threadIdx.x; e < total; e += (int64_t)gridDim.x * blockDim.x) {
    const int t = (int)(e & 3);
    const int l = (int)((e >> 2) & 63);
    const int64_t blk = e >> 8;
    float v = 0.f;
    if (!d.transposed) {
      const int KS = d.n_cols / 8;
      const int nt = (int)(blk / KS), ks = (int)(blk % KS);
      const int n = nt * 32 + (l & 31);
      const int kp = ks * 8 + (l >> 5) * 4 + t;
      int col = -1;
      if (kp < d.segA_pad) {
        if (kp < d.segA_valid) col = kp;
      } else {
        const int q = kp - d.segA_pad;
        if (q < d.segB_valid) col = d.segA_valid + q;
      }
      if (col >= 0) v = src[(int64_t)n * d.ld + col];
    } else {
      const int KS = d.n_rows / 8;
      const int jt = (int)(blk / KS), ks = (int)(blk % KS);
      const int o = ks * 8 + (l >> 5) * 4 + t;
      const int c = d.col0 + jt * 32 + (l & 31);
      v = src[(int64_t)o * d.ld + c];
    }
    dst[e] = v;
  }
}

__global__ void __launch_bounds__(256) pack6_kernel(PackTable tab, const float* __restrict__ params,
                                                     uint4* __restrict__ pf, uint4* __restrict__ pb) {
  const PackDesc d = tab.d[blockIdx.y];
  constexpr int TW = 16, KW = 32;
  const int KS = (d.transposed ? d.n_rows : d.n_cols) / KW;
  const int NTL = (d.transposed ? d.n_cols : d.n_rows) / TW;
  const int64_t total = (int64_t)NTL * KS * 64;
  uint4* dst = (d.transposed ? pb : pf) + d.dst_off * 3 / 8;
  const float* src = params + d.src_off;
  for (int64_t e = blockIdx.x * (int64_t)blockDim.x + threadIdx.x; e < total; e += (int64_t)gridDim.x * blockDim.x) {
    const int l = (int)(e & 63);
    const int64_t blk = e >> 6;
    const int tile = (int)(blk / KS), ks = (int)(blk % KS);
    float v[8];
#pragma unroll
    for (int j = 0; j < 8; ++j) {
      const int kp = ks * KW + (l / TW) * 8 + j;
      v[j] = 0.f;
      if (!d.transposed) {
        const int n = tile * TW + (l % TW);
        int col = -1;
        if (kp < d.segA_pad) { if (kp < d.segA_valid) col = kp; }
        else { const int q = kp - d.segA_pad; if (q < d.segB_valid) col = d.segA_valid + q; }
        if (col >= 0) v[j] = src[(int64_t)n * d.ld + col];
      } else {
        v[j] = src[(int64_t)kp * d.ld + d.col0 + tile * TW + (l % TW)];
      }
    }
    unsigned h[4], m[4], lo[4];
#pragma unroll
    for (int q = 0; q < 4; ++q) {
      split3_pair(v[2 * q], v[2 * q + 1], h[q], m[q], lo[q]);
    }
    uint4* o = dst + (blk * 3) * 64 + l;
    o[0] = make_uint4(h[0], h[1], h[2], h[3]);
    o[64] = make_uint4(m[0], m[1], m[2], m[3]);
    o[128] = make_uint4(lo[0], lo[1], lo[2], lo[3]);
  }
}

static PackTable make_pack_table(const NetLayout& L) {
  PackTable T;
  int n = 0;
  for (int l = 0; l < 8; ++l) {
    PackDesc d{};
    d.src_off = L.LW[l]; d.dst_off = L.PF[l]; d.n_rows = 256;
    d.ld = (l == 0) ? L.in_pe : (l == 5 ? 256 + L.in_pe : 256);
    d.n_cols = (l == 0) ? L.pe_pad : (l == 5 ? L.pe_pad + 256 : 256);
    if (l == 0) { d.segA_pad = L.pe_pad; d.segA_valid = L.in_pe; d.segB_valid = 0; }
    else if (l == 5) { d.segA_pad = L.pe_pad; d.segA_valid = L.in_pe; d.segB_valid = 256; }
    else { d.segA_pad = 256; d.segA_valid = 256; d.segB_valid = 0; }
    T.d[n++] = d;
  }
  { PackDesc d{}; d.src_off = L.FW; d.dst_off = L.PF[8]; d.ld = 256; d.n_rows = 256; d.n_cols = 256;
    d.segA_pad = 256; d.segA_valid = 256; T.d[n++] = d; }
  { PackDesc d{}; d.src_off = L.VW; d.dst_off = L.PF[9]; d.ld = 283; d.n_rows = 128; d.n_cols = 288;
    d.segA_pad = 256; d.segA_valid = 256; d.segB_valid = 27; T.d[n++] = d; }
  { PackDesc d{}; d.transposed = 1; d.src_off = L.VW; d.dst_off = L.PB[0]; d.ld = 283; d.n_rows = 128; d.n_cols = 256; d.col0 = 0; T.d[n++] = d; }
  { PackDesc d{}; d.transposed = 1; d.src_off = L.FW; d.dst_off = L.PB[1]; d.ld = 256; d.n_rows = 256; d.n_cols = 256; d.col0 = 0; T.d[n++] = d; }
  const int order[7] = {7, 6, 5, 4, 3, 2, 1};
  for (int j = 0; j < 7; ++j) {
    const int l = order[j];
    PackDesc d{}; d.transposed = 1; d.src_off = L.LW[l]; d.dst_off = L.PB[2 + j]; d.n_rows = 256; d.n_cols = 256;
    d.ld = (l == 5) ? 256 + L.in_pe : 256;
    d.col0 = (l == 5) ? L.in_pe : 0;
    T.d[n++] = d;
  }
  return T;
}


extern "C" int64_t fastnerf_net_floats(int kind, int what) {
  if (kind < 0 || kind > 2) return -1;
  const NetLayout& L = layout_of(kind);
  return what == 0 ? L.n_params : what == 1 ? L.pf_total : what == 2 ? L.pb_total : what == 3 ? L.pe_pad : -1;
}
extern "C" int64_t fastnerf_mlp_act_floats(int kind, int64_t P) {
  if (kind < 0 || kind > 2 || P < 0) return -1;
  return act_floats(P, layout_of(kind).pe_pad);
}

extern "C" int fastnerf_mlp_pack_ex(int kind, const float* params, float* packed_fwd, float* packed_bwd,
                                    fn_stream_t stream) {
  FN_CHECK_ARG(kind >= 0 && kind <= 2 && params && packed_fwd && packed_bwd, "kind in 0..2, non-null pointers");
  static const PackTable T[3] = {make_pack_table(layout_of(0)), make_pack_table(layout_of(1)),
                                 make_pack_table(layout_of(2))};
  hipLaunchKernelGGL(pack_kernel, dim3(64, 19), dim3(256), 0, fn::S(stream), T[kind], params, packed_fwd, packed_bwd);
  FN_LAUNCH_CHECK();
  return 0;
}
extern "C" int64_t fastnerf_mlp_x6_packed_floats(int kind, int which) {
  if (kind < 0 || kind > 2 || (which != 1 && which != 2)) return -1;
  const NetLayout& L = layout_of(kind);
  return (which == 1 ? L.pf_total : L.pb_total) * 3 / 2;
}
extern "C" int fastnerf_mlp_x6_pack(int kind, const float* params, float* packed_fwd, float* packed_bwd, fn_stream_t stream) {
  FN_CHECK_ARG(kind >= 0 && kind <= 2 && params && packed_fwd && packed_bwd, "kind in 0..2, non-null pointers");
  static const PackTable T[3] = {make_pack_table(layout_of(0)), make_pack_table(layout_of(1)),
                                 make_pack_table(layout_of(2))};
  hipLaunchKernelGGL(pack6_kernel, dim3(32, 19), dim3(256), 0, fn::S(stream), T[kind], params,
                     reinterpret_cast<uint4*>(packed_fwd), reinterpret_cast<uint4*>(packed_bwd));
  FN_LAUNCH_CHECK();
  return 0;
}
extern "C" int fastnerf_mlp_pack(const float* params, float* packed_fwd, float* packed_bwd, fn_stream_t stream) {
  return fastnerf_mlp_pack_ex(0, params, packed_fwd, packed_bwd, stream);
}
```

include/fastnerf.h:

```cpp
#ifndef FASTNERF_H
#define FASTNERF_H
#include <stdint.h>
#ifdef __cplusplus
extern "C" {
#endif

typedef void* fn_stream_t;

int fastnerf_version(void);
const char* fastnerf_last_error(void);
int fastnerf_device_cus(void);

int fastnerf_gen_rays(int H, int W, float fx, float fy, float cx, float cy, const float* c2w_host,
                      float* rays_o, float* rays_d, fn_stream_t stream);
int fastnerf_gen_rays_pixels(int64_t n, const int32_t* pix, const float* poses, float fx, float fy, float cx,
                             float cy, float* rays_o, float* rays_d, fn_stream_t stream);
int fastnerf_ndc_rays(int64_t n, int H, int W, double focal, float near, const float* rays_o, const float* rays_d,
                      float* out_o, float* out_d, fn_stream_t stream);
int fastnerf_pack_rays(int64_t n, const float* rays_o, const float* rays_d, float near, float far, int ndc, int H,
                       int W, double focal, float* rays11, fn_stream_t stream);
int fastnerf_sample_coarse(int64_t n, int S, const float* rays11, int lindisp, int perturb, const float* t_rand,
                           uint64_t seed, float* z, fn_stream_t stream);
int fastnerf_posenc(int64_t n, int L, const float* x, float* out, fn_stream_t stream);

#define FASTNERF_NET_PARAMS 595844
#define FASTNERF_PACKED_FWD 593920
#define FASTNERF_PACKED_BWD 557056
#define FASTNERF_ACT_FLOATS 2592
#define FASTNERF_ACT_SLACK 8192
#define FASTNERF_DACT_FLOATS 2432

int fastnerf_mlp_pack(const float* params, float* packed_fwd, float* packed_bwd, fn_stream_t stream);
int fastnerf_mlp_fwd(int64_t n, int S, const float* rays11, const float* z, const float* params,
                     const float* packed_fwd, float* raw, float* act, fn_stream_t stream);
int64_t fastnerf_mlp_bwd_partial_floats(void);
int fastnerf_mlp_bwd(int64_t n, int S, const float* draw, const float* act, const float* params,
                     const float* packed_bwd, float* dact, float* partial, float* grads, fn_stream_t stream);

int fastnerf_raw2outputs_fwd(int64_t n, int S, const float* raw, const float* z, const float* rays11,
                             const float* noise, int white_bkgd, float* rgb_map, float* disp, float* acc,
                             float* weights, float* depth, fn_stream_t stream);
int fastnerf_raw2outputs_bwd(int64_t n, int S, const float* raw, const float* z, const float* rays11,
                             const float* noise, int white_bkgd, const float* g_rgb, float* draw,
                             fn_stream_t stream);
int fastnerf_raw2outputs_bwd_full(int64_t n, int S, const float* raw, const float* z, const float* rays11,
                                  const float* noise, int white_bkgd, const float* acc, const float* depth,
                                  const float* g_rgb, const float* g_disp, const float* g_acc, const float* g_w,
                                  const float* g_depth, float* draw, fn_stream_t stream);
int fastnerf_sample_pdf_merge(int64_t n, int S, int Ni, const float* z, const float* weights, int det,
                              const float* u, uint64_t seed, float* z_out, float* z_samples, float* z_std,
                              fn_stream_t stream);

int fastnerf_sample_pdf(int64_t n, int M, int Ni, const float* bins, const float* weights, int det, const float* u,
                        uint64_t seed, float* samples, fn_stream_t stream);

int fastnerf_mse_leafmax(int64_t n, const float* rgb, const float* rgb0, const float* target, float grad_scale,
                         float* g_rgb, float* g_rgb0, float* loss2, const int32_t* leaf_tag, int max_leaves,
                         uint32_t* table, fn_stream_t stream);
int fastnerf_adam_step(int64_t n, float* params, const float* grads, float* m, float* v, double lr, double beta1,
                       double beta2, double eps, int step, fn_stream_t stream);

int64_t fastnerf_net_floats(int kind, int what);
int64_t fastnerf_mlp_act_floats(int kind, int64_t n_points);
int fastnerf_mlp_pack_ex(int kind, const float* params, float* packed_fwd, float* packed_bwd, fn_stream_t stream);
int fastnerf_mlp_fwd_ex(int kind, int64_t n, int S, const float* rays11, const float* z, const float* params,
                        const float* packed_fwd, float* raw, float* act, fn_stream_t stream);
int fastnerf_mlp_bwd_ex(int kind, int64_t n, int S, const float* draw, const float* act, const float* params,
                        const float* packed_bwd, float* dact, float* partial, float* grads, fn_stream_t stream);

int64_t fastnerf_mlp_bf16_floats(int kind, int what, int64_t n_points);
int64_t fastnerf_mlp_bf16_partial_floats(void);
int fastnerf_mlp_bf16_pack(int kind, const float* params, float* packed_fwd, float* packed_bwd, fn_stream_t stream);
int fastnerf_mlp_bf16_fwd(int kind, int64_t n, int S, const float* rays11, const float* z, const float* params,
                          const float* packed_fwd, float* raw, float* act, fn_stream_t stream);
int fastnerf_mlp_bf16_bwd(int kind, int64_t n, int S, const float* draw, const float* act, const float* params,
                          const float* packed_bwd, float* dact, float* partial, float* grads, fn_stream_t stream);

#define FN_FWD_SKIP_DEAD_RGB 1
int fastnerf_mlp_bf16_fwd_flags(int kind, int64_t n, int S, const float* rays11, const float* z, const float* params,
                                const float* packed_fwd, float* raw, int flags, fn_stream_t stream);
int fastnerf_mlp_fwd_flags_ex(int kind, int64_t n, int S, const float* rays11, const float* z, const float* params,
                              const float* packed_fwd, float* raw, int flags, fn_stream_t stream);

int fastnerf_render_rays_fwd(int math_mode, int64_t n, int N_samples, int N_importance, const float* rays11, int lindisp,
                             int perturb, int det, int white_bkgd, const float* t_rand, const float* u,
                             const float* noise0, const float* noise1, uint64_t seed0, uint64_t seed1,
                             const float* params_c, const float* packed_c, const float* params_f, const float* packed_f,
                             float* z0, float* raw0, float* act0, float* rgb0, float* disp0, float* acc0, float* w0,
                             float* depth0, float* z1, float* z_samples, float* z_std, float* raw1, float* act1,
                             float* rgb1, float* disp1, float* acc1, float* w1, float* depth1, fn_stream_t stream);
int fastnerf_render_rays_fwd_ex(int math_mode, int64_t n, int N_samples, int N_importance, const float* rays11, int lindisp,
                                int perturb, int det, int white_bkgd, const float* t_rand, const float* u,
                                const float* noise0, const float* noise1, uint64_t seed0, uint64_t seed1,
                                const float* params_c, const float* packed_c, const float* params_f, const float* packed_f,
                                float* z0, float* raw0, float* act0, float* rgb0, float* disp0, float* acc0, float* w0,
                                float* depth0, float* z1, float* z_samples, float* z_std, float* raw1, float* act1,
                                float* rgb1, float* disp1, float* acc1, float* w1, float* depth1, int flags, fn_stream_t stream);

int fastnerf_render_rays_bwd(int math_mode, int64_t n, int N_samples, int N_importance, const float* rays11, int white_bkgd,
                             const float* g_rgb, const float* g_rgb0, const float* noise0, const float* noise1,
                             const float* z0, const float* raw0, const float* act0, const float* z1, const float* raw1,
                             const float* act1, const float* params_c, const float* packed_bwd_c, const float* params_f,
                             const float* packed_bwd_f, float* draw_ws, float* dact_ws, float* partial_ws, float* grads_c,
                             float* grads_f, fn_stream_t stream);

int fastnerf_pp_gen_rays(int H, int W, const double* intrinsics_host, const double* c2w_host, float* rays_o,
                         float* rays_d, fn_stream_t stream);
int fastnerf_leaf_sumcount(int64_t n, const float* rgb, const float* target, const int32_t* leaf_tag, int max_leaves,
                           double* sum, int32_t* count, fn_stream_t stream);
int fastnerf_pp_intersect_sphere(int64_t n, const float* rays11, float* fg_far, int* n_outside, fn_stream_t stream);
int fastnerf_pp_fg_depths(int64_t n, int S, float near, const float* fg_far, int perturb, const float* t_rand,
                          uint64_t seed, float* z, fn_stream_t stream);
int fastnerf_pp_sample_pdf_merge(int64_t n, int S, int Ni, const float* z, const float* weights, int det,
                                 const float* u, uint64_t seed, float* z_out, float* z_samples, fn_stream_t stream);
int fastnerf_pp_perturb_samples(int64_t n, int S, const float* z_in, const float* t_rand, uint64_t seed, float* z_out,
                                fn_stream_t stream);
int fastnerf_pp_sample_pdf(int64_t n, int M, int Ni, const float* bins, const float* weights, int det, const float* u,
                           uint64_t seed, float* samples, fn_stream_t stream);
int fastnerf_pp_depth2pts_outside(int64_t n, int S, const float* ray_o, const float* ray_d, const float* depth, float* pts,
                                  float* depth_real, fn_stream_t stream);
int fastnerf_pp_composite_fwd(int64_t n, int S, int part, const float* raw, const float* z, const float* rays11,
                              const float* fg_far, float* rgb_map, float* weights, float* depth, float* lambda,
                              fn_stream_t stream);
int fastnerf_pp_composite_bwd(int64_t n, int S, int part, const float* raw, const float* z, const float* rays11,
                              const float* fg_far, const float* g_rgb, const float* g_lambda, float* draw,
                              fn_stream_t stream);

typedef struct fn_tree fn_tree;
fn_tree* fastnerf_tree_create(int H, int W, int n_images, int max_depth);
void fastnerf_tree_destroy(fn_tree* t);
int fastnerf_tree_num_leaves(const fn_tree* t, int image);
int fastnerf_tree_max_leaves(const fn_tree* t);
double fastnerf_tree_min_area(const fn_tree* t, int image);
int fastnerf_tree_get_leaves(const fn_tree* t, int image, double* out_host);
int fastnerf_tree_set_leaves(fn_tree* t, int image, int n_leaves, const double* boxes_host, double min_area);
int fastnerf_tree_leaf_plan(const fn_tree* t, int image, double ray_num_per_pixel, int last_epoch,
                            int32_t* out_host);
int64_t fastnerf_tree_adjust(fn_tree* t, const float* table_host, int max_leaves, double thres);
int64_t fastnerf_tree_adjust_mean(fn_tree* t, const double* sum_host, const int32_t* count_host, int max_leaves,
                                  double thres);


int64_t fastnerf_tree_epoch_plan(const fn_tree* t, double ray_num_per_pixel, int last_epoch, int32_t* out_host,
                                 int64_t* n_rays_host);
int fastnerf_epoch_rays(int64_t N, int L, const int32_t* plan, const int64_t* offs, const float* images,
                        const float* poses, int n_img, int H, int W, float fx, float fy, float cx, float cy,
                        uint64_t seed, int shuffle, const int32_t* n_weighted, const int64_t* seg_beg,
                        const int64_t* seg_end, const int32_t* order, const double* cum, float* rays_o, float* rays_d,
                        float* rgb, int32_t* tag, int32_t* pix, fn_stream_t stream);
int64_t fastnerf_epoch_shard_rows(int64_t N, int64_t batch, int row0, int stride);
int fastnerf_epoch_rays_shard(int64_t N, int L, const int32_t* plan, const int64_t* offs, const float* images,
                              const float* poses, int n_img, int H, int W, float fx, float fy, float cx, float cy,
                              uint64_t seed, int shuffle, const int32_t* n_weighted, const int64_t* seg_beg,
                              const int64_t* seg_end, const int32_t* order, const double* cum, int64_t batch, int row0, int stride,
                              float* rays_o, float* rays_d, float* rgb, int32_t* tag, int32_t* pix, fn_stream_t stream);

int fastnerf_gauss_noise(int64_t n, float std, uint64_t seed, float* out, fn_stream_t stream);

int64_t fastnerf_compact_ws_ints(int64_t n_points);
int fastnerf_compact_live(int64_t n_points, const float* draw, int32_t* live_idx, int32_t* count_out, int32_t* ws,
                          fn_stream_t stream);
int fastnerf_mlp_bf16_fwd_live(int kind, int64_t n, int S, const float* rays11, const float* z, const float* params,
                               const float* packed_fwd, float* act, const int32_t* live_idx, const int32_t* live_cnt,
                               fn_stream_t stream);
int fastnerf_mlp_bf16_bwd_live(int kind, int64_t n, int S, const float* draw, const float* act, const float* params,
                               const float* packed_bwd, float* dact, float* partial, float* grads,
                               const int32_t* live_idx, const int32_t* live_cnt, fn_stream_t stream);
int fastnerf_mlp_fwd_live_ex(int kind, int64_t n, int S, const float* rays11, const float* z, const float* params,
                             const float* packed_fwd, float* act, const int32_t* live_idx, const int32_t* live_cnt,
                             fn_stream_t stream);
int fastnerf_mlp_bwd_live_ex(int kind, int64_t n, int S, const float* draw, const float* act, const float* params,
                             const float* packed_bwd, float* dact, float* partial, float* grads,
                             const int32_t* live_idx, const int32_t* live_cnt, fn_stream_t stream);
int fastnerf_render_rays_bwd_live(int math_mode, int64_t n, int N_samples, int N_importance, const float* rays11, int white_bkgd,
                                  const float* g_rgb, const float* g_rgb0, const float* noise0, const float* noise1,
                                  const float* z0, const float* raw0, const float* z1, const float* raw1,
                                  const float* params_c, const float* packed_fwd_c, const float* packed_bwd_c,
                                  const float* params_f, const float* packed_fwd_f, const float* packed_bwd_f,
                                  float* draw_ws, float* act_ws, float* dact_ws, float* partial_ws, int32_t* live_ws,
                                  float* grads_c, float* grads_f, int32_t* counts_out, fn_stream_t stream);

int64_t fastnerf_mlp_x6_packed_floats(int kind, int which);
int fastnerf_mlp_x6_pack(int kind, const float* params, float* packed_fwd, float* packed_bwd, fn_stream_t stream);
int fastnerf_mlp_x6_fwd(int kind, int64_t n, int S, const float* rays11, const float* z, const float* params,
                        const float* packed_fwd, float* raw, float* act, int flags, fn_stream_t stream);
int fastnerf_mlp_x6_bwd(int kind, int64_t n, int S, const float* draw, const float* act, const float* params,
                        const float* packed_bwd, float* dact, float* partial, float* grads, fn_stream_t stream);
int fastnerf_mlp_x6_fwd_live(int kind, int64_t n, int S, const float* rays11, const float* z, const float* params,
                             const float* packed_fwd, float* act, const int32_t* live_idx, const int32_t* live_cnt,
                             fn_stream_t stream);
int fastnerf_mlp_x6_bwd_live(int kind, int64_t n, int S, const float* draw, const float* act, const float* params,
                             const float* packed_bwd, float* dact, float* partial, float* grads, const int32_t* live_idx,
                             const int32_t* live_cnt, fn_stream_t stream);

#define FN_STEP_FORWARD 1
#define FN_STEP_BWD_FINE 2
#define FN_STEP_BWD_COARSE 4
#define FN_STEP_UPDATE 8
struct fn_occ_grid;
typedef struct fn_step_args {
  int64_t n;
  const float *rays_o, *rays_d, *target;
  const float *t_rand, *u, *noise0, *noise1;
  uint64_t seed0, seed1;
  const int32_t* leaf_tag;
  uint32_t* table;
  int64_t net_floats;
  float *params, *grads, *adam_m, *adam_v;
  float *packed_fwd_c, *packed_bwd_c, *packed_fwd_f, *packed_bwd_f;
  float *rays11, *z0, *raw0, *act0, *rgb0, *disp0, *acc0, *w0, *depth0;
  float *z1, *z_samples, *z_std, *raw1, *act1, *rgb1, *disp1, *acc1, *w1, *depth1;
  float *g_rgb, *g_rgb0, *loss2;
  float *draw_ws, *act_ws, *dact_ws, *partial_ws;
  int32_t *live_ws, *counts;
  double focal, lr, beta1, beta2, eps;
  float near_plane, far_plane, grad_scale;
  int32_t math_mode;
  int32_t N_samples, N_importance, lindisp, perturb, white_bkgd, ndc, H, W;
  int32_t live;
  int32_t fwd_flags;
  int32_t max_leaves, adam_t;
  const struct fn_occ_grid* occ;
  int32_t* occ_counts;
} fn_step_args;
int64_t fastnerf_step_args_size(void);
int fastnerf_train_step(const fn_step_args* args, int phases, fn_stream_t stream);

#define FASTNERF_COMM_ID_BYTES 128
typedef struct fn_comm fn_comm;
int fastnerf_comm_unique_id(char* id);
int fastnerf_comm_init(fn_comm** out, const char* id, int rank, int world);
int fastnerf_comm_destroy(fn_comm* comm);
int fastnerf_allreduce_grads(fn_comm* comm, float* grads, int64_t n, float scale, fn_stream_t stream);
int fastnerf_allreduce_leaf_table(fn_comm* comm, uint32_t* table, int64_t n, fn_stream_t stream);
int fastnerf_allreduce_leaf_sumcount(fn_comm* comm, double* sum, int32_t* count, int64_t n, fn_stream_t stream);
int fastnerf_leaf_table_reset(uint32_t* table, int64_t n, fn_stream_t stream);
int fastnerf_leaf_table_read(const uint32_t* table, float* host_out, int64_t n, fn_stream_t stream);

#define FASTNERF_MC_TRI_STRIDE 16
int fastnerf_grid_points(int64_t p0, int64_t n, const float* xs, int64_t nx, const float* ys, int64_t ny, const float* zs,
                         int64_t nz, float* rays11, fn_stream_t stream);
int fastnerf_grid_sigma(int64_t n, const float* raw, float* out, fn_stream_t stream);
int64_t fastnerf_mc_ws_bytes(int64_t nx, int64_t ny, int64_t nz);
int fastnerf_mc_count(const float* vol, int64_t nx, int64_t ny, int64_t nz, float thr, void* ws, int64_t* counts_host,
                      fn_stream_t stream);
int fastnerf_mc_emit(const float* vol, int64_t nx, int64_t ny, int64_t nz, float thr, void* ws, float* verts, int32_t* tris,
                     fn_stream_t stream);
int fastnerf_mc_tables(int8_t* tri_host, uint16_t* edge_host);


typedef struct fn_occ_grid {
  const uint32_t* words;
  float lo[3], inv[3];
  int32_t n[3];
  int32_t outside_occupied;
} fn_occ_grid;
int64_t fastnerf_occ_words(int64_t nx, int64_t ny, int64_t nz);
int fastnerf_occ_build(const float* vol, int64_t nx, int64_t ny, int64_t nz, float threshold, int dilate, uint32_t* words,
                       uint32_t* ws, fn_stream_t stream);
int fastnerf_occ_from_mask(const uint8_t* mask, int64_t nx, int64_t ny, int64_t nz, uint32_t* words, fn_stream_t stream);
int fastnerf_occ_query(const fn_occ_grid* grid, int64_t n, const float* pts, uint8_t* out, fn_stream_t stream);
int fastnerf_occ_classify(const fn_occ_grid* grid, int64_t n, int S, const float* rays11, const float* z, int32_t* live_idx,
                          int32_t* count_out, float* raw, int32_t* ws, fn_stream_t stream);
#define FN_OCC_MAX_LEVELS 8
typedef struct fn_occ_cascade {
  int32_t levels;
  int32_t reserved;
  fn_occ_grid level[FN_OCC_MAX_LEVELS];
} fn_occ_cascade;
int fastnerf_occ_query_cascade(const fn_occ_cascade* cascade, int64_t n, const float* pts, uint8_t* out, fn_stream_t stream);
int fastnerf_occ_classify_cascade(const fn_occ_cascade* cascade, int64_t n, int S, const float* rays11, const float* z,
                                  int32_t* live_idx, int32_t* count_out, float* raw, int32_t* ws, fn_stream_t stream);
int fastnerf_occ_cell_points(const fn_occ_grid* grid, int64_t c0, int64_t n, uint64_t seed, float* rays11, fn_stream_t stream);
int fastnerf_occ_update(const float* raw_c, const float* raw_f, int64_t c0, int64_t n, int64_t nx, int64_t ny, int64_t nz,
                        float decay, float threshold, int dilate, float* dens, uint32_t* words, uint32_t* ws, fn_stream_t stream);
int fastnerf_mlp_fwd_list_ex(int kind, int64_t n, int S, const float* rays11, const float* z, const float* params,
                             const float* packed_fwd, float* raw, const int32_t* live_idx, const int32_t* live_cnt, int flags,
                             fn_stream_t stream);
int fastnerf_mlp_bf16_fwd_list(int kind, int64_t n, int S, const float* rays11, const float* z, const float* params,
                               const float* packed_fwd, float* raw, const int32_t* live_idx, const int32_t* live_cnt, int flags,
                               fn_stream_t stream);
int fastnerf_mlp_x6_fwd_list(int kind, int64_t n, int S, const float* rays11, const float* z, const float* params,
                             const float* packed_fwd, float* raw, const int32_t* live_idx, const int32_t* live_cnt, int flags,
                             fn_stream_t stream);
int fastnerf_render_rays_fwd_occ(int math_mode, int64_t n, int N_samples, int N_importance, const float* rays11, int lindisp,
                                 int perturb, int det, int white_bkgd, const float* t_rand, const float* u, uint64_t seed0,
                                 uint64_t seed1, const float* params_c, const float* packed_c, const float* params_f,
                                 const float* packed_f, const fn_occ_grid* grid, int32_t* live_ws, int32_t* counts_out, float* z0,
                                 float* raw0, float* rgb0, float* disp0, float* acc0, float* w0, float* depth0, float* z1,
                                 float* z_samples, float* z_std, float* raw1, float* rgb1, float* disp1, float* acc1, float* w1,
                                 float* depth1, int flags, fn_stream_t stream);
int fastnerf_render_rays_fwd_occ_cascade(int math_mode, int64_t n, int N_samples, int N_importance, const float* rays11, int lindisp,
                                         int perturb, int det, int white_bkgd, const float* t_rand, const float* u, uint64_t seed0,
                                         uint64_t seed1, const float* params_c, const float* packed_c, const float* params_f,
                                         const float* packed_f, const fn_occ_cascade* cascade, int32_t* live_ws, int32_t* counts_out,
                                         float* z0, float* raw0, float* rgb0, float* disp0, float* acc0, float* w0, float* depth0,
                                         float* z1, float* z_samples, float* z_std, float* raw1, float* rgb1, float* disp1,
                                         float* acc1, float* w1, float* depth1, int flags, fn_stream_t stream);

int64_t fastnerf_mlp_sigma_grad_ws_floats(int math_mode, int64_t n_points);
int fastnerf_mlp_sigma_grad(int math_mode, int kind, int64_t n, int S, const float* rays11, const float* z, const float* params,
                            const float* packed_fwd, const float* packed_bwd, float* ws, float* sigma, float* grad,
                            fn_stream_t stream);

#ifdef __cplusplus
}
#endif
#endif
```

Baseline: 229,300 rays/s.

## Fold the linear feature layer into the view layer weights

The linear feature layer (FW/FB, no activation) is algebraically merged into the first view-branch layer. A folded weight matrix and bias are precomputed at pack time in a per-packed-buffer side allocation. The forward pass drops the 256x256 feature GEMM and applies the folded weights directly to h7. In backward, the dx chain uses the folded matrix, and the dW for the view layer is taken against h7. A new unfold kernel then recovers the FW/FB/VW gradients through small double-precision matmuls. This removes one large GEMM per point in both forward and backward, at the cost of extra pack-time work, a global map keyed by buffer address, and small per-step unfold kernels with possible numerical differences.

```diff
diff --git a/fast-learning-nerf_amd/_lib.py b/fast-learning-nerf_amd/_lib.py
--- a/fast-learning-nerf_amd/_lib.py
+++ b/fast-learning-nerf_amd/_lib.py
@@ -113,6 +113,8 @@
     'fastnerf_render_rays_bwd_live': (I, [I, L, I, I, P, I] + [P] * 22 + [P]),
     'fastnerf_mlp_x6_packed_floats': (L, [I, I]),
     'fastnerf_mlp_x6_pack': (I, [I, P, P, P, P]),
+    'fastnerf_mlp_fold_buffer': (P, [P]),
+    'fastnerf_mlp_fold_offset': (L, [I, I]),
     'fastnerf_mlp_x6_fwd': (I, [I, L, I, P, P, P, P, P, P, I, P]),
     'fastnerf_mlp_x6_bwd': (I, [I, L, I, P, P, P, P, P, P, P, P]),
     'fastnerf_mlp_x6_fwd_live': (I, [I, L, I, P, P, P, P, P, P, P, P]),
diff --git a/fast-learning-nerf_amd/csrc/mlp_bwd_dw.hip b/fast-learning-nerf_amd/csrc/mlp_bwd_dw.hip
--- a/fast-learning-nerf_amd/csrc/mlp_bwd_dw.hip
+++ b/fast-learning-nerf_amd/csrc/mlp_bwd_dw.hip
@@ -180,7 +180,6 @@
   for (int k = 0; k < TPW; ++k) ssum[k] = 0.f;
 
   constexpr int CTI1 = CTI - CTI2, KI1 = CTI1 * 32, KI2 = CTI2 * 32;
-  static_assert(!(RANK1 && CTI2), "the rank-1 row is taken over X only");
   constexpr int CTO1 = CTO - CTO2, NO1 = CTO1 * 32, NO2 = CTO2 * 32;
   static_assert(!(RANK1 && CTO2) && !(CTI2 && CTO2), "one second tensor per job");
   const float* tsrc[TPW];
@@ -267,7 +266,7 @@
         split3_frag(make_float4(v[0], v[1], v[2], v[3]), make_float4(v[4], v[5], v[6], v[7]), h, m, l);
         d[0] = h; d[64] = m; d[128] = l;
         if (BIAS && (KNOWN ? (k * NW < CTO) : (t < CTO1))) ssum[k] += ((v[0] + v[1]) + (v[2] + v[3])) + ((v[4] + v[5]) + (v[6] + v[7]));
-        if (RANK1 && (KNOWN ? (k * NW >= CTO) : (t >= CTO))) {
+        if (RANK1 && (KNOWN ? (k * NW >= CTO) : (t >= CTO && t < CTO + CTI1))) {
           const float4 d0 = *reinterpret_cast<const float4*>(DA + (st & 1) * 16 + half8);
           const float4 d1 = *reinterpret_cast<const float4*>(DA + (st & 1) * 16 + half8 + 4);
           const float da[8] = {d0.x, d0.y, d0.z, d0.w, d1.x, d1.y, d1.z, d1.w};
@@ -374,7 +373,7 @@
         const float sv = ssum[k] + __shfl_xor(ssum[k], 32, 64);
         if (lane < 32) {
           if (BIAS && t < CTO1) partial_b[(int64_t)wg * NO1 + t * 32 + lane] = sv;
-          if (RANK1 && t >= CTO) partial_r[(int64_t)wg * KI + (t - CTO) * 32 + lane] = sv;
+          if (RANK1 && t >= CTO && t < CTO + CTI1) partial_r[(int64_t)wg * KI1 + (t - CTO) * 32 + lane] = sv;
         }
       }
     }
@@ -400,24 +399,21 @@
   k = k < 1 ? 1 : (k > 8 ? 8 : k);
   return unit * (int)k;
 }
+#define DW_TRUNK_JOBS 7
 struct DwTrunk {
-  const float* dY[8];
-  const float* X[8];
-  float* pw[8];
-  float* pb[8];
+  const float* dY[DW_TRUNK_JOBS];
+  const float* X[DW_TRUNK_JOBS];
+  float* pw[DW_TRUNK_JOBS];
+  float* pb[DW_TRUNK_JOBS];
 };
 __global__ void __launch_bounds__(512, 2)
-mlp_bwd_dw6_trunk_kernel(int64_t P, DwTrunk J, const float* __restrict__ draw, float* __restrict__ partial_r,
-                         const int* __restrict__ live_idx, const int* __restrict__ live_cnt, int ncu) {
+mlp_bwd_dw6_trunk_kernel(int64_t P, DwTrunk J, const int* __restrict__ live_idx, const int* __restrict__ live_cnt, int ncu) {
   if (live_idx) P = (int64_t)__builtin_amdgcn_readfirstlane(*live_cnt);
   const int nact = dw_trunk_chunks(P, ncu);
   if ((int)blockIdx.x >= nact) return;
   const int job = (int)blockIdx.y;
-  if (job == 7)
-    dw6_body<4, 2, 2, 4, true, true>(P, J.dY[7], J.X[7], draw, J.pw[7], J.pb[7], partial_r, live_idx, nullptr, nullptr, (int)blockIdx.x, nact);
-  else
-    dw6_body<4, 2, 2, 4, true, false>(P, J.dY[job], J.X[job], nullptr, J.pw[job], J.pb[job], nullptr, live_idx, nullptr, nullptr,
-                                      (int)blockIdx.x, nact);
+  dw6_body<4, 2, 2, 4, true, false>(P, J.dY[job], J.X[job], nullptr, J.pw[job], J.pb[job], nullptr, live_idx, nullptr, nullptr,
+                                    (int)blockIdx.x, nact);
 }
 
 __global__ void __launch_bounds__(128) head_grads_kernel(int64_t P, const float* __restrict__ draw,
@@ -465,6 +461,8 @@
   int64_t dst;
   int nwg, rows, cols, ld, valid_cols;
   int dyn;
+  int sc_cols;
+  int64_t sc_dst;
 };
 #define MAX_SEGS 32
 struct RedTable {
@@ -472,8 +470,8 @@
   int n;
 };
 
-__global__ void __launch_bounds__(256) reduce_all_kernel(RedTable tab, const float* __restrict__ partial,
-                                                          float* __restrict__ grads, int64_t P, const int* __restrict__ live_cnt, int ncu) {
+__global__ void __launch_bounds__(256) reduce_all_kernel(RedTable tab, const float* __restrict__ partial, float* __restrict__ grads,
+                                                          float* __restrict__ scratch, int64_t P, const int* __restrict__ live_cnt, int ncu) {
   RedSeg sg = tab.s[blockIdx.y];
   if (sg.dyn) {
     if (live_cnt) P = (int64_t)*live_cnt;
@@ -501,8 +499,42 @@
     for (int h = RS / 2; h >= 1; h >>= 1)
 #pragma unroll
       for (int i = 0; i < h; ++i) a[i] += a[i + h];
-    grads[sg.dst + (int64_t)r * sg.ld + c] = a[0];
-  }
+    if (c < sg.sc_cols) scratch[sg.sc_dst + (int64_t)r * sg.sc_cols + c] = a[0];
+    else grads[sg.dst + (int64_t)r * sg.ld + c] = a[0];
+  }
+}
+
+__global__ void __launch_bounds__(256) unfold_kernel(const float* __restrict__ G, const float* __restrict__ params, float* __restrict__ grads,
+                                                      int64_t VW, int64_t VB, int64_t FW, int64_t FB) {
+  __shared__ double As[16][17], Bs[16][17];
+  const int tx = threadIdx.x & 15, ty = threadIdx.x >> 4;
+  const int b = blockIdx.x;
+  if (b == 384) {
+    const int i = threadIdx.x;
+    double s = 0.0;
+    for (int o = 0; o < 128; ++o) s = fma((double)params[VW + (int64_t)o * 283 + i], (double)grads[VB + o], s);
+    grads[FB + i] = (float)s;
+    return;
+  }
+  const bool wf = b < 256;
+  const int r0 = wf ? (b >> 4) * 16 : ((b - 256) >> 4) * 16, c0 = (b & 15) * 16;
+  const int K = wf ? 128 : 256;
+  double s = 0.0;
+  for (int k0 = 0; k0 < K; k0 += 16) {
+    if (wf) {
+      As[ty][tx] = (double)params[VW + (int64_t)(k0 + ty) * 283 + r0 + tx];
+      Bs[ty][tx] = (double)G[(k0 + ty) * 256 + c0 + tx];
+    } else {
+      As[tx][ty] = (double)G[(r0 + ty) * 256 + k0 + tx];
+      Bs[tx][ty] = (double)params[FW + (int64_t)(c0 + ty) * 256 + k0 + tx];
+    }
+    __syncthreads();
+#pragma unroll
+    for (int k = 0; k < 16; ++k) s = fma(As[k][ty], Bs[k][tx], s);
+    __syncthreads();
+  }
+  if (wf) grads[FW + (int64_t)(r0 + ty) * 256 + c0 + tx] = (float)s;
+  else grads[VW + (int64_t)(r0 + ty) * 283 + c0 + tx] = (float)fma((double)grads[VB + r0 + ty], (double)params[FB + c0 + tx], s);
 }
 
 struct DwJobDesc { int NO, KI, bias, rank1; };
@@ -537,11 +569,11 @@
 template <int WO, int WI, int TO, int TI, bool BIAS, bool RANK1, int MM = MM_F32, int CTI2 = 0, int CTO2 = 0>
 static int launch_dw(int64_t P, const float* dY, int ldy, const float* X, int ldx, const float* draw, float* base,
                      int nwg, hipStream_t st, const int* live_idx = nullptr, const int* live_cnt = nullptr,
-                     const float* X2 = nullptr, const float* dY2 = nullptr) {
+                     const float* X2 = nullptr, const float* dY2 = nullptr, float* pr_at = nullptr) {
   constexpr int NO = WO * TO * 32, KI = WI * TI * 32;
   float* pw = base;
   float* pb = base + (int64_t)nwg * NO * KI;
-  float* pr = pb + (BIAS ? (int64_t)nwg * (NO - CTO2 * 32) : 0);
+  float* pr = pr_at ? pr_at : pb + (BIAS ? (int64_t)nwg * (NO - CTO2 * 32) : 0);
   if constexpr (MM == MM_X6) {
     if (ldy != NO - CTO2 * 32 || ldx != KI - CTI2 * 32 || (CTI2 > 0) != (X2 != nullptr) || (CTO2 > 0) != (dY2 != nullptr)) {
       fn::set_error("launch_dw: the bf16x6 dW kernel needs ld == width (and X2 / dY2 exactly when CTI2 / CTO2 > 0)");
@@ -574,10 +606,10 @@
 }
 
 static void add_seg(RedTable& T, int64_t src, int64_t wg_stride, int nwg, int rows, int cols, int64_t dst, int ld,
-                    int valid_cols, int dyn = 0) {
+                    int valid_cols, int dyn = 0, int sc_cols = 0, int64_t sc_dst = 0) {
   RedSeg& s = T.s[T.n++];
   s.src = src; s.wg_stride = wg_stride; s.nwg = nwg; s.rows = rows; s.cols = cols; s.dst = dst; s.ld = ld;
-  s.valid_cols = valid_cols; s.dyn = dyn;
+  s.valid_cols = valid_cols; s.dyn = dyn; s.sc_cols = sc_cols; s.sc_dst = sc_dst;
 }
 
 template <int MM>
@@ -637,40 +669,40 @@
   }
   if constexpr (MW == MM_X6) {
     DwTrunk J;
-    for (int l = 1; l <= 8; ++l) {
-      const int j = l < 8 ? l : 9;
-      J.dY[l - 1] = l < 8 ? dact + dact_y(P, l) : dact + dact_feat(P);
+    for (int l = 1; l < 8; ++l) {
+      J.dY[l - 1] = dact + dact_y(P, l);
       J.X[l - 1] = act + act_h(P, PEP, l - 1);
-      J.pw[l - 1] = region(j);
-      J.pb[l - 1] = region(j) + (int64_t)nwg * 256 * 256;
-    }
-    float* pr = J.pb[7] + (int64_t)nwg * 256;
+      J.pw[l - 1] = region(l);
+      J.pb[l - 1] = region(l) + (int64_t)nwg * 256 * 256;
+    }
     constexpr int lds6 = 2 * 16 * 3 * 1024 + 128;
     static bool attr_t = false;
     if (!attr_t) {
       FN_HIP(hipFuncSetAttribute(reinterpret_cast<const void*>(mlp_bwd_dw6_trunk_kernel), hipFuncAttributeMaxDynamicSharedMemorySize, lds6));
       attr_t = true;
     }
-    hipLaunchKernelGGL(mlp_bwd_dw6_trunk_kernel, dim3(dw_trunk_chunks(P, ncu), 8), dim3(512), lds6, st, P, J, draw, pr, live_idx, live_cnt, ncu);
+    hipLaunchKernelGGL(mlp_bwd_dw6_trunk_kernel, dim3(dw_trunk_chunks(P, ncu), DW_TRUNK_JOBS), dim3(512), lds6, st, P, J, live_idx, live_cnt, ncu);
     FN_LAUNCH_CHECK();
     for (int l = 1; l < 8; ++l) segs(l, L.LW[l] + (l == 5 ? L.in_pe : 0), l == 5 ? 256 + L.in_pe : 256, 256, L.LB[l], 0, 1);
-    segs(9, L.FW, 256, 256, L.FB, L.AW, 1);
-  } else {
-    if ((rc = launch_dw<4, 2, 2, 4, true, true, MW>(P, dact + dact_feat(P), 256, act + act_h(P, PEP, 7), 256, draw, region(9), nwg, st, live_idx, live_cnt))) return rc;
-    segs(9, L.FW, 256, 256, L.FB, L.AW);
-  }
+  }
+  float* const pr_view = region(9);
+  const int64_t g_off = dw_job_base(9, ncu, PEP) + (int64_t)nwg * 256;
   if constexpr (MW == MM_X6) {
-    if ((rc = launch_dw<4, 3, 1, 3, true, false, MW, 1, 0>(P, dact + dact_yv(P), 128, act + act_feat(P, PEP), 256, nullptr, region(10), nwg, st,
-                                                     live_idx, live_cnt, act + act_vpe(P, PEP), nullptr))) return rc;
+    if ((rc = launch_dw<4, 3, 1, 3, true, true, MW, 1, 0>(P, dact + dact_yv(P), 128, act + act_h(P, PEP, 7), 256, draw, region(10), nwg, st,
+                                                    live_idx, live_cnt, act + act_vpe(P, PEP), nullptr, pr_view))) return rc;
     const int64_t b10 = dw_job_base(10, ncu, PEP);
-    add_seg(T, b10, 128 * 288, nwg, 128, 288, L.VW, 283, 283);
+    add_seg(T, b10, 128 * 288, nwg, 128, 288, L.VW, 283, 283, 0, 256, g_off);
     add_seg(T, b10 + (int64_t)nwg * 128 * 288, 128, nwg, 1, 128, L.VB, 128, 128);
   } else {
-    if ((rc = launch_dw<2, 4, 2, 2, true, false, MW>(P, dact + dact_yv(P), 128, act + act_feat(P, PEP), 256, nullptr, region(10), nwg, st, live_idx, live_cnt))) return rc;
-    segs(10, L.VW, 283, 256, L.VB, 0);
+    if ((rc = launch_dw<2, 4, 2, 2, true, true, MW>(P, dact + dact_yv(P), 128, act + act_h(P, PEP, 7), 256, draw, region(10), nwg, st, live_idx, live_cnt,
+                                              nullptr, nullptr, pr_view))) return rc;
+    const int64_t b10 = dw_job_base(10, ncu, PEP);
+    add_seg(T, b10, 128 * 256, nwg, 128, 256, L.VW, 283, 256, 0, 256, g_off);
+    add_seg(T, b10 + (int64_t)nwg * 128 * 256, 128, nwg, 1, 128, L.VB, 128, 128);
     if ((rc = launch_dw<4, 1, 1, 1, false, false, MW>(P, dact + dact_yv(P), 128, act + act_vpe(P, PEP), 32, nullptr, region(11), nwg, st, live_idx, live_cnt))) return rc;
     segs(11, L.VW + 256, 283, 27, 0, 0);
   }
+  add_seg(T, dw_job_base(9, ncu, PEP), 256, nwg, 1, 256, L.AW, 256, 256);
   {
     const int hg = HEAD_MAX_WG;
     const int64_t hb = dw_job_base(12, ncu, PEP);
@@ -679,7 +711,9 @@
     add_seg(T, hb, 388, hg, 1, 388, L.RW, 388, 387);
     add_seg(T, hb + 387, 388, hg, 1, 1, L.AB, 1, 1);
   }
-  hipLaunchKernelGGL(reduce_all_kernel, dim3(256, T.n), dim3(256), 0, st, T, partial, grads, P, live_cnt, ncu);
+  hipLaunchKernelGGL(reduce_all_kernel, dim3(256, T.n), dim3(256), 0, st, T, partial, grads, partial, P, live_cnt, ncu);
+  FN_LAUNCH_CHECK();
+  hipLaunchKernelGGL(unfold_kernel, dim3(385), dim3(256), 0, st, partial + g_off, params, grads, L.VW, L.VB, L.FW, L.FB);
   FN_LAUNCH_CHECK();
   return 0;
 }
diff --git a/fast-learning-nerf_amd/csrc/mlp_bwd_dx.hip b/fast-learning-nerf_amd/csrc/mlp_bwd_dx.hip
--- a/fast-learning-nerf_amd/csrc/mlp_bwd_dx.hip
+++ b/fast-learning-nerf_amd/csrc/mlp_bwd_dx.hip
@@ -143,17 +143,9 @@
     AccT<L16, 2> acc;
     WRegsT<L16, 2> wch;
     zero_acc<2>(acc);
-    gemm<MM, 2, 0>(acc, Hs, 0, 16, wblock<MM>(packed_t, lay.PB[0]), 16, 0, wn * 2, wm, lane);
-    __syncthreads();
-    wprefetch(wch, wblock<MM>(packed_t, lay.PB[1]), 32, 0, 32, wn * 2, lane);
-    epilogue_dx<false, false>(acc, Hs, Es, dx_preload<false, false, L16>(nullptr, nullptr, wn, lane), nullptr, wm, wn, lane,
-                              valid);
-    __syncthreads();
-    zero_acc<2>(acc);
     {
       const DxPre pre = dx_preload<true, true, L16>(maskw + (7 * NWAVES + wave) * 64, params + lay.AW, wn, lane);
-      gemm<MM, 2, 0, CHAIN>(acc, Hs, 0, 32, wblock<MM>(packed_t, lay.PB[1]), 32, 0, wn * 2, wm, lane, 0,
-                            dact + dact_feat(PL) + p0 * 256, valid, wave, wch);
+      gemm<MM, 2, 0>(acc, Hs, 0, 16, wblock<MM>(packed_t, lay.PBM), 16, 0, wn * 2, wm, lane);
       __syncthreads();
       wprefetch(wch, wblock<MM>(packed_t, lay.PB[2]), 32, 0, 32, wn * 2, lane);
       epilogue_dx<true, true>(acc, Hs, Es, pre, nullptr, wm, wn, lane, valid);
diff --git a/fast-learning-nerf_amd/csrc/mlp_fwd.hip b/fast-learning-nerf_amd/csrc/mlp_fwd.hip
--- a/fast-learning-nerf_amd/csrc/mlp_fwd.hip
+++ b/fast-learning-nerf_amd/csrc/mlp_fwd.hip
@@ -1,4 +1,6 @@
 #include "mlp_common.h"
+
+float* fn_fold_buffer(const float* packed_fwd, bool create);
 
 __device__ __forceinline__ void bg_point(const float* __restrict__ o, const float* __restrict__ d, float depth,
                                          float x[4]) {
@@ -39,8 +41,8 @@
 template <bool SAVE, bool BG, int MM = MM_F32, bool LIST = false>
 __global__ void __launch_bounds__(NTHR, 2 * NTHR / 512 * WG_PER_CU)
 mlp_fwd_kernel(int64_t P, int S, const float* __restrict__ rays, const float* __restrict__ zv,
-               const float* __restrict__ params, const float* __restrict__ packed, float* __restrict__ raw,
-               float* __restrict__ act, NetLayout lay, unsigned* __restrict__ sched, const int* __restrict__ live_idx,
+               const float* __restrict__ params, const float* __restrict__ packed, const float* __restrict__ fold,
+               float* __restrict__ raw, float* __restrict__ act, NetLayout lay, unsigned* __restrict__ sched, const int* __restrict__ live_idx,
                const int* __restrict__ live_cnt, int flags) {
   const int64_t PL = P;
   if (live_idx) P = (int64_t)__builtin_amdgcn_readfirstlane(*live_cnt);
@@ -208,12 +210,6 @@
     if (skip_tail) {
       if (pq == 0 && pm < valid && raw) *reinterpret_cast<float4*>(raw + (LIST ? pp : p0 + pm) * 4) = make_float4(0.f, 0.f, 0.f, alpha_val);
     } else {
-    load_bias<2>(bv2, params + lay.FB, wn, lane);
-    init_acc<2, FOLD>(acc, bv2);
-    gemm<MM, 2, 0>(acc, Hs, 0, 32, wblock<MM>(packed, lay.PF[8]), 32, 0, wn * 2, wm, lane, dbg,
-                   SAVE ? act + act_h(PL, PEP, 7) + p0 * 256 : nullptr, valid, wave);
-    __syncthreads();
-    epilogue_fwd<2, false, false, FOLD>(acc, bv2, Hs, wm, wn, lane, nullptr, 256, valid);
     __syncthreads();
     if (SAVE) {
       float* avp = act + act_vpe(PL, PEP) + p0 * 32;
@@ -226,11 +222,11 @@
     {
       AccT<L16, 1> av;
       float bv1[L16 ? 2 : 1];
-      load_bias<1>(bv1, params + lay.VB, wn, lane);
+      load_bias<1>(bv1, fold + fold_plain(lay.PFB, L16), wn, lane);
       init_acc<1, FOLD>(av, bv1);
-      gemm<MM, 1, 0>(av, Hs, 0, 32, wblock<MM>(packed, lay.PF[9]), 36, 0, wn, wm, lane, dbg,
-                     SAVE ? act + act_feat(PL, PEP) + p0 * 256 : nullptr, valid, wave);
-      gemm<MM, 1, 1>(av, Es, 0, 4, wblock<MM>(packed, lay.PF[9]), 36, 32, wn, wm, lane, dbg);
+      gemm<MM, 1, 0>(av, Hs, 0, 32, wblock<MM>(fold, lay.PFM), 36, 0, wn, wm, lane, dbg,
+                     SAVE ? act + act_h(PL, PEP, 7) + p0 * 256 : nullptr, valid, wave);
+      gemm<MM, 1, 1>(av, Es, 0, 4, wblock<MM>(fold, lay.PFM), 36, 32, wn, wm, lane, dbg);
       __syncthreads();
       epilogue_fwd<1, true, false, FOLD>(av, bv1, Hs, wm, wn, lane, nullptr, 128, valid);
       __syncthreads();
@@ -282,7 +278,9 @@
     FN_HIP(hipFuncSetAttribute(reinterpret_cast<const void*>(kern), hipFuncAttributeMaxDynamicSharedMemorySize, LDS_BYTES));
     attr = true;
   }
-  hipLaunchKernelGGL(kern, dim3(grid), dim3(NTHR), LDS_BYTES, st, P, S, rays11, z, params, packed_fwd, raw, act, lay, sched, live_idx,
+  const float* fold = fn_fold_buffer(packed_fwd, false);
+  FN_CHECK_ARG(fold != nullptr, "packed_fwd was not filled by a pack call of this process (the folded view layer is kept by its address)");
+  hipLaunchKernelGGL(kern, dim3(grid), dim3(NTHR), LDS_BYTES, st, P, S, rays11, z, params, packed_fwd, fold, raw, act, lay, sched, live_idx,
                      live_cnt, flags);
   FN_LAUNCH_CHECK();
   return 0;
diff --git a/fast-learning-nerf_amd/csrc/mlp_layout.h b/fast-learning-nerf_amd/csrc/mlp_layout.h
--- a/fast-learning-nerf_amd/csrc/mlp_layout.h
+++ b/fast-learning-nerf_amd/csrc/mlp_layout.h
@@ -6,6 +6,7 @@
   int64_t LW[8], LB[8];
   int64_t VW, VB, FW, FB, AW, AB, RW, RB;
   int64_t PF[10], PB[9];
+  int64_t PFM, PFB, PFR, PBM, fold_total;
   int64_t n_params, pf_total, pb_total;
   int in_pe, pe_pad;
   int kind;
@@ -36,10 +37,18 @@
   }
   L.pf_total = p;
   p = 0;
+  L.PFM = p; p += (int64_t)288 * 128;
+  L.PFB = p; p += 128;
+  L.PFR = p; p += (int64_t)128 * 256;
+  L.fold_total = p;
+  p = 0;
   for (int j = 0; j < 9; ++j) { L.PB[j] = p; p += (int64_t)(j == 0 ? 128 : 256) * 256; }
+  L.PBM = p; p += (int64_t)128 * 256;
   L.pb_total = p;
   return L;
 }
+
+inline __host__ __device__ int64_t fold_plain(int64_t off, bool x6) { return x6 ? off * 3 / 2 : off; }
 
 constexpr int ACT_REST = 8 * 256 + 256 + 32 + 128;
 constexpr int ACT_MASK = 64;
diff --git a/fast-learning-nerf_amd/csrc/mlp_pack.hip b/fast-learning-nerf_amd/csrc/mlp_pack.hip
--- a/fast-learning-nerf_amd/csrc/mlp_pack.hip
+++ b/fast-learning-nerf_amd/csrc/mlp_pack.hip
@@ -1,4 +1,7 @@
 #include "mlp_common.h"
+#include <map>
+#include <mutex>
+#include <utility>
 
 struct PackDesc {
   int64_t src_off;
@@ -9,17 +12,59 @@
   int segA_pad, segA_valid, segB_valid;
   int col0;
   int transposed;
+  int fold;
 };
+#define N_PACK 21
 struct PackTable {
-  PackDesc d[19];
+  PackDesc d[N_PACK];
+  int64_t m_off;
 };
 
+__global__ void __launch_bounds__(256) fold_kernel(const float* __restrict__ params, int64_t VW, int64_t VB, int64_t FW, int64_t FB,
+                                                    float* __restrict__ m_out, float* __restrict__ b_out) {
+  const int e = blockIdx.x * 256 + threadIdx.x;
+  if (e < 128 * 256) {
+    const int o = e >> 8, j = e & 255;
+    const float* wv = params + VW + (int64_t)o * 283;
+    const float* wf = params + FW + j;
+    double s = 0.0;
+#pragma unroll 8
+    for (int i = 0; i < 256; ++i) s = fma((double)wv[i], (double)wf[(int64_t)i * 256], s);
+    m_out[e] = (float)s;
+  } else if (e < 128 * 256 + 128) {
+    const int o = e - 128 * 256;
+    const float* wv = params + VW + (int64_t)o * 283;
+    double s = (double)params[VB + o];
+    for (int i = 0; i < 256; ++i) s = fma((double)wv[i], (double)params[FB + i], s);
+    b_out[o] = (float)s;
+  }
+}
+static void launch_fold(const NetLayout& L, const float* params, float* fold, bool x6, hipStream_t st) {
+  hipLaunchKernelGGL(fold_kernel, dim3(129), dim3(256), 0, st, params, L.VW, L.VB, L.FW, L.FB, fold + fold_plain(L.PFR, x6),
+                     fold + fold_plain(L.PFB, x6));
+}
+static std::mutex g_fold_mu;
+static std::map<std::pair<int, const void*>, float*> g_fold;
+float* fn_fold_buffer(const float* packed_fwd, bool create) {
+  int dev = 0;
+  if (hipGetDevice(&dev) != hipSuccess) return nullptr;
+  std::lock_guard<std::mutex> lk(g_fold_mu);
+  auto it = g_fold.find({dev, packed_fwd});
+  if (it != g_fold.end()) return it->second;
+  if (!create) return nullptr;
+  float* p = nullptr;
+  if (hipMalloc(reinterpret_cast<void**>(&p), sizeof(float) * (size_t)(layout_of(0).fold_total * 3 / 2)) != hipSuccess) return nullptr;
+  g_fold[{dev, packed_fwd}] = p;
+  return p;
+}
+
 __global__ void __launch_bounds__(256) pack_kernel(PackTable tab, const float* __restrict__ params,
-                                                    float* __restrict__ pf, float* __restrict__ pb) {
+                                                    float* __restrict__ pf, float* __restrict__ pb, float* fold) {
   const PackDesc d = tab.d[blockIdx.y];
   const int64_t total = (int64_t)d.n_rows * d.n_cols;
-  float* dst = (d.transposed ? pb : pf) + d.dst_off;
+  float* dst = (d.transposed ? pb : (d.fold ? fold : pf)) + d.dst_off;
   const float* src = params + d.src_off;
+  const float* mraw = fold + tab.m_off;
   for (int64_t e = blockIdx.x * (int64_t)blockDim.x + threadIdx.x; e < total; e += (int64_t)gridDim.x * blockDim.x) {
     const int t = (int)(e & 3);
     const int l = (int)((e >> 2) & 63);
@@ -37,27 +82,28 @@
         const int q = kp - d.segA_pad;
         if (q < d.segB_valid) col = d.segA_valid + q;
       }
-      if (col >= 0) v = src[(int64_t)n * d.ld + col];
+      if (col >= 0) v = (d.fold && kp < d.segA_pad) ? mraw[n * 256 + col] : src[(int64_t)n * d.ld + col];
     } else {
       const int KS = d.n_rows / 8;
       const int jt = (int)(blk / KS), ks = (int)(blk % KS);
       const int o = ks * 8 + (l >> 5) * 4 + t;
       const int c = d.col0 + jt * 32 + (l & 31);
-      v = src[(int64_t)o * d.ld + c];
+      v = d.fold ? mraw[o * 256 + c] : src[(int64_t)o * d.ld + c];
     }
     dst[e] = v;
   }
 }
 
 __global__ void __launch_bounds__(256) pack6_kernel(PackTable tab, const float* __restrict__ params,
-                                                     uint4* __restrict__ pf, uint4* __restrict__ pb) {
+                                                     uint4* __restrict__ pf, uint4* __restrict__ pb, uint4* fold) {
   const PackDesc d = tab.d[blockIdx.y];
   constexpr int TW = 16, KW = 32;
   const int KS = (d.transposed ? d.n_rows : d.n_cols) / KW;
   const int NTL = (d.transposed ? d.n_cols : d.n_rows) / TW;
   const int64_t total = (int64_t)NTL * KS * 64;
-  uint4* dst = (d.transposed ? pb : pf) + d.dst_off * 3 / 8;
+  uint4* dst = (d.transposed ? pb : (d.fold ? fold : pf)) + d.dst_off * 3 / 8;
   const float* src = params + d.src_off;
+  const float* mraw = reinterpret_cast<const float*>(fold) + tab.m_off;
   for (int64_t e = blockIdx.x * (int64_t)blockDim.x + threadIdx.x; e < total; e += (int64_t)gridDim.x * blockDim.x) {
     const int l = (int)(e & 63);
     const int64_t blk = e >> 6;
@@ -72,9 +118,10 @@
         int col = -1;
         if (kp < d.segA_pad) { if (kp < d.segA_valid) col = kp; }
         else { const int q = kp - d.segA_pad; if (q < d.segB_valid) col = d.segA_valid + q; }
-        if (col >= 0) v[j] = src[(int64_t)n * d.ld + col];
+        if (col >= 0) v[j] = (d.fold && kp < d.segA_pad) ? mraw[n * 256 + col] : src[(int64_t)n * d.ld + col];
       } else {
-        v[j] = src[(int64_t)kp * d.ld + d.col0 + tile * TW + (l % TW)];
+        const int c = d.col0 + tile * TW + (l % TW);
+        v[j] = d.fold ? mraw[kp * 256 + c] : src[(int64_t)kp * d.ld + c];
       }
     }
     unsigned h[4], m[4], lo[4];
@@ -89,8 +136,9 @@
   }
 }
 
-static PackTable make_pack_table(const NetLayout& L) {
+static PackTable make_pack_table(const NetLayout& L, bool x6) {
   PackTable T;
+  T.m_off = fold_plain(L.PFR, x6);
   int n = 0;
   for (int l = 0; l < 8; ++l) {
     PackDesc d{};
@@ -116,6 +164,9 @@
     d.col0 = (l == 5) ? L.in_pe : 0;
     T.d[n++] = d;
   }
+  { PackDesc d{}; d.fold = 1; d.src_off = L.VW; d.dst_off = L.PFM; d.ld = 283; d.n_rows = 128; d.n_cols = 288;
+    d.segA_pad = 256; d.segA_valid = 256; d.segB_valid = 27; T.d[n++] = d; }
+  { PackDesc d{}; d.fold = 1; d.transposed = 1; d.src_off = L.VW; d.dst_off = L.PBM; d.ld = 256; d.n_rows = 128; d.n_cols = 256; d.col0 = 0; T.d[n++] = d; }
   return T;
 }
 
@@ -133,9 +184,13 @@
 extern "C" int fastnerf_mlp_pack_ex(int kind, const float* params, float* packed_fwd, float* packed_bwd,
                                     fn_stream_t stream) {
   FN_CHECK_ARG(kind >= 0 && kind <= 2 && params && packed_fwd && packed_bwd, "kind in 0..2, non-null pointers");
-  static const PackTable T[3] = {make_pack_table(layout_of(0)), make_pack_table(layout_of(1)),
-                                 make_pack_table(layout_of(2))};
-  hipLaunchKernelGGL(pack_kernel, dim3(64, 19), dim3(256), 0, fn::S(stream), T[kind], params, packed_fwd, packed_bwd);
+  static const PackTable T[3] = {make_pack_table(layout_of(0), false), make_pack_table(layout_of(1), false),
+                                 make_pack_table(layout_of(2), false)};
+  float* fold = fn_fold_buffer(packed_fwd, true);
+  FN_CHECK_ARG(fold != nullptr, "buffer of the folded view layer (hipMalloc failed?)");
+  launch_fold(layout_of(kind), params, fold, false, fn::S(stream));
+  FN_LAUNCH_CHECK();
+  hipLaunchKernelGGL(pack_kernel, dim3(64, N_PACK), dim3(256), 0, fn::S(stream), T[kind], params, packed_fwd, packed_bwd, fold);
   FN_LAUNCH_CHECK();
   return 0;
 }
@@ -146,13 +201,25 @@
 }
 extern "C" int fastnerf_mlp_x6_pack(int kind, const float* params, float* packed_fwd, float* packed_bwd, fn_stream_t stream) {
   FN_CHECK_ARG(kind >= 0 && kind <= 2 && params && packed_fwd && packed_bwd, "kind in 0..2, non-null pointers");
-  static const PackTable T[3] = {make_pack_table(layout_of(0)), make_pack_table(layout_of(1)),
-                                 make_pack_table(layout_of(2))};
-  hipLaunchKernelGGL(pack6_kernel, dim3(32, 19), dim3(256), 0, fn::S(stream), T[kind], params,
-                     reinterpret_cast<uint4*>(packed_fwd), reinterpret_cast<uint4*>(packed_bwd));
+  static const PackTable T[3] = {make_pack_table(layout_of(0), true), make_pack_table(layout_of(1), true),
+                                 make_pack_table(layout_of(2), true)};
+  float* fold = fn_fold_buffer(packed_fwd, true);
+  FN_CHECK_ARG(fold != nullptr, "buffer of the folded view layer (hipMalloc failed?)");
+  launch_fold(layout_of(kind), params, fold, true, fn::S(stream));
+  FN_LAUNCH_CHECK();
+  hipLaunchKernelGGL(pack6_kernel, dim3(32, N_PACK), dim3(256), 0, fn::S(stream), T[kind], params,
+                     reinterpret_cast<uint4*>(packed_fwd), reinterpret_cast<uint4*>(packed_bwd), reinterpret_cast<uint4*>(fold));
   FN_LAUNCH_CHECK();
   return 0;
 }
 extern "C" int fastnerf_mlp_pack(const float* params, float* packed_fwd, float* packed_bwd, fn_stream_t stream) {
   return fastnerf_mlp_pack_ex(0, params, packed_fwd, packed_bwd, stream);
 }
+
+
+extern "C" const float* fastnerf_mlp_fold_buffer(const float* packed_fwd) { return fn_fold_buffer(packed_fwd, false); }
+extern "C" int64_t fastnerf_mlp_fold_offset(int kind, int what) {
+  if (kind < 0 || kind > 2) return -1;
+  const NetLayout& L = layout_of(kind);
+  return what == 0 ? L.PFM : what == 1 ? L.PFB : what == 2 ? L.PFR : what == 3 ? L.PBM : what == 4 ? L.fold_total : -1;
+}
diff --git a/include/fastnerf.h b/include/fastnerf.h
--- a/include/fastnerf.h
+++ b/include/fastnerf.h
@@ -182,6 +182,8 @@
 
 int64_t fastnerf_mlp_x6_packed_floats(int kind, int which);
 int fastnerf_mlp_x6_pack(int kind, const float* params, float* packed_fwd, float* packed_bwd, fn_stream_t stream);
+const float* fastnerf_mlp_fold_buffer(const float* packed_fwd);
+int64_t fastnerf_mlp_fold_offset(int kind, int what);
 int fastnerf_mlp_x6_fwd(int kind, int64_t n, int S, const float* rays11, const float* z, const float* params,
                         const float* packed_fwd, float* raw, float* act, int flags, fn_stream_t stream);
 int fastnerf_mlp_x6_bwd(int kind, int64_t n, int S, const float* draw, const float* act, const float* params,
```

Measured after the change: 249,200 rays/s (median of 6 runs). 8.6% higher.
